# rbitr/llm.f90

Measured on AMD Instinct MI355X. Metric: tokens/sec TinyLlama-1.1B decode, higher is better.
Workload: dtype f32; 1 GPU; tinyllama f32 decode, greedy, positions 6..1140 (./llm -n 1140 -t 0); consumer=logits to host + host argmax (llmk_forward), parallelism=single GPU, seed=20260928

## Files before the change

### include/llmk.h

```cpp
#ifndef LLMK_H
#define LLMK_H

#include <stddef.h>
#include <stdint.h>

#ifdef __cplusplus
extern "C" {
#endif

#define LLMK_TYPE_F32 0
#define LLMK_TYPE_F16 1
#define LLMK_TYPE_Q4_0 2
#define LLMK_TYPE_Q6_K 14

#define LLMK_TOKEN_EMBEDDING_TABLE 0
#define LLMK_RMS_ATT_WEIGHT 1
#define LLMK_RMS_FFN_WEIGHT 2
#define LLMK_WQKV 3
#define LLMK_WO 4
#define LLMK_W13 5
#define LLMK_W2 6
#define LLMK_RMS_FINAL_WEIGHT 7
#define LLMK_WCLS 8
#define LLMK_N_TENSORS 9

#define LLMK_FLAG_NO_GRAPH 1
#define LLMK_FLAG_TIMINGS 2
#define LLMK_FLAG_MULTI_KERNEL 4

#define LLMK_OK 0
#define LLMK_E_ARG 1
#define LLMK_E_SHAPE 2
#define LLMK_E_SIZE 3
#define LLMK_E_TYPE 4
#define LLMK_E_STATE 5
#define LLMK_E_NODEVICE 6
#define LLMK_E_NOMEM 7
#define LLMK_E_TIMEOUT 8
#define LLMK_E_COMM 9
#define LLMK_E_VERIFY 10
#define LLMK_E_NONFINITE 11
#define LLMK_E_HIP 1000

typedef struct llmk_config {
    int32_t emb_dim;
    int32_t hidden_dim;
    int32_t n_layers;
    int32_t n_heads;
    int32_t n_kv_heads;
    int32_t vocab_size;
    int32_t seq_len;
    int32_t weight_type;
    int32_t device;
    int32_t flags;
} llmk_config;

typedef struct llmk_ctx llmk_ctx;

int llmk_create(const llmk_config *cfg, llmk_ctx **out);

int llmk_create_tp(const llmk_config *cfg, int tp_rank, int tp_size, llmk_ctx **out);
int llmk_tp_unique_id(char id_out[128]);
int llmk_tp_init_comm(llmk_ctx *ctx, const char id[128]);

int llmk_tp_p2p_handle(llmk_ctx *ctx, char handle_out[64]);
int llmk_tp_p2p_connect(llmk_ctx *ctx, const char *handles);
int llmk_tp_p2p_connect_local(llmk_ctx *ctx, llmk_ctx *const *ranks);
int llmk_tp_p2p_selftest(llmk_ctx *ctx, int iters);
int llmk_tp_p2p_stress(llmk_ctx *ctx, int iters, unsigned seed);
int llmk_tp_p2p_disable(llmk_ctx *ctx);

int llmk_tp_begin(llmk_ctx *ctx, int token, int pos);
int llmk_tp_segment(llmk_ctx *ctx, int seg, int layer);
int llmk_tp_read_partial(llmk_ctx *ctx, float *out);
int llmk_tp_write_partial(llmk_ctx *ctx, const float *in);
int llmk_tp_read_logits(llmk_ctx *ctx, float *out_slice);

int llmk_upload(llmk_ctx *ctx, int tensor_id, const void *host, size_t nbytes, int ggml_type);

int llmk_upload_rows(llmk_ctx *ctx, int tensor_id, int layer, int row_offset, int rows, const void *host,
                     size_t nbytes, int ggml_type);

int llmk_set_tensor_type(llmk_ctx *ctx, int tensor_id, int ggml_type);
int llmk_set_rms_eps(llmk_ctx *ctx, float eps);

int llmk_set_rope_freqs(llmk_ctx *ctx, const float *freqs, int n);

int llmk_forward(llmk_ctx *ctx, int token, int pos, float *logits_out);

int llmk_prefill(llmk_ctx* ctx, const int* tokens, int n, int pos0, float* logits_out);

int llmk_score(llmk_ctx *ctx, const int *tokens, int n, int pos0, const int *targets, float *logprob_out, int *argmax_out,
               float *logits_out);

int llmk_forward_greedy(llmk_ctx *ctx, int token, int pos, int *next_token);

typedef void (*llmk_token_fn)(int index, int token, void *user);
int llmk_decode_greedy(llmk_ctx *ctx, int token, int pos0, int n, int *ids_out, llmk_token_fn on_token, void *user);

int llmk_forward_sample(llmk_ctx *ctx, int token, int pos, float temperature, uint64_t seed, int *next_token);
int llmk_decode_sample(llmk_ctx *ctx, int token, int pos0, int n, float temperature, uint64_t seed,
                       int *ids_out, llmk_token_fn on_token, void *user);

typedef struct llmk_sampler {
    float temperature;
    int32_t top_k;
    float top_p;
    float min_p;
    uint64_t seed;
} llmk_sampler;
int llmk_forward_sample_ex(llmk_ctx *ctx, int token, int pos, const llmk_sampler *sampler, int *next_token);
int llmk_decode_sample_ex(llmk_ctx *ctx, int token, int pos0, int n, const llmk_sampler *sampler, int *ids_out,
                          llmk_token_fn on_token, void *user);
int llmk_sample_logits(llmk_ctx *ctx, const float *logits, int pos, const llmk_sampler *sampler, int *token_out, int *kept_out,
                       float *tau_out);

#define LLMK_MAX_LOGIT_BIAS 256
typedef struct llmk_logit_bias { int32_t token; float bias; } llmk_logit_bias;
typedef struct llmk_penalties {
    int32_t last_n;
    float repeat;
    float frequency;
    float presence;
    const llmk_logit_bias *bias; int32_t n_bias;
} llmk_penalties;
int llmk_set_history(llmk_ctx *ctx, const int *tokens, int n, int pos0);
int llmk_get_history(llmk_ctx *ctx, int *tokens_out, int n, int pos0);
int llmk_forward_sample_pen(llmk_ctx *ctx, int token, int pos, const llmk_sampler *sampler, const llmk_penalties *penalties, int *next_token);
int llmk_decode_sample_pen(llmk_ctx *ctx, int token, int pos0, int n, const llmk_sampler *sampler, const llmk_penalties *penalties,
                           int *ids_out, llmk_token_fn on_token, void *user);
int llmk_sample_logits_pen(llmk_ctx *ctx, const float *logits, int pos, const llmk_sampler *sampler, const llmk_penalties *penalties,
                           int *token_out, int *kept_out, float *tau_out, float *adjusted_out);

#define LLMK_MAX_TOP_LOGPROBS 20
typedef struct llmk_logprobs {
    int32_t top_n;
    float *token_logprob;
    int32_t *top_tokens;
    float *top_logprobs;
} llmk_logprobs;
int llmk_forward_sample_lp(llmk_ctx *ctx, int token, int pos, const llmk_sampler *sampler, const llmk_penalties *penalties,
                           const llmk_logprobs *logprobs, int *next_token);
int llmk_decode_sample_lp(llmk_ctx *ctx, int token, int pos0, int n, const llmk_sampler *sampler, const llmk_penalties *penalties,
                          const llmk_logprobs *logprobs, int *ids_out, llmk_token_fn on_token, void *user);
int llmk_logprob_logits(llmk_ctx *ctx, const float *logits, int token, int top_n, float *token_logprob, int32_t *top_tokens,
                        float *top_logprobs);

typedef struct llmk_batch llmk_batch;
#define LLMK_MAX_BATCH 128
int llmk_batch_create(llmk_ctx *ctx, int n_slots, int seq_len, llmk_batch **out);
int llmk_batch_destroy(llmk_batch *b);
int llmk_batch_fork(llmk_batch *b, int slot, int n_pos);
int llmk_batch_forward(llmk_batch *b, int n, const int *slots, const int *tokens, const int *pos, float *logits_out, int *argmax_out);
int llmk_batch_decode(llmk_batch *b, int n, const int *slots, const int *tokens, const int *pos0, int steps,
                      const llmk_sampler *samplers, int *ids_out);
int llmk_batch_time(llmk_batch *b, int n, int pos, int iters, float *avg_ms);

int llmk_rows_set_history(llmk_batch *b, int slot, const int *tokens, int n, int pos0);
int llmk_rows_get_history(llmk_batch *b, int slot, int *tokens_out, int n, int pos0);
int llmk_rows_decode(llmk_batch *b, int n, const int *slots, const int *tokens, const int *pos0, int steps,
                     const llmk_sampler *samplers, const llmk_penalties *penalties, const llmk_logprobs *logprobs, int *ids_out);
int llmk_rows_sample_logits(llmk_batch *b, int n, const int *slots, const int *pos, const float *logits,
                            const llmk_sampler *samplers, const llmk_penalties *penalties, const llmk_logprobs *logprobs,
                            int *tokens_out, int *kept_out, float *tau_out, float *adjusted_out);

int llmk_prefix_set(llmk_batch *b, int n_pos);
int llmk_prefix_attach(llmk_batch *b, int slot);
int llmk_prefix_len(llmk_batch *b);

int llmk_reset(llmk_ctx *ctx);

// ... 35 lines not shown
```

### llm.f90_amd/csrc/llmk.hip

```cpp
#include "../../include/llmk.h"
#include "kernels.h"
#include "token_kernel.h"
#include "prefill.h"
#include "batch.h"
#include "tp_p2p.h"

#include <rccl/rccl.h>

#include <algorithm>
#include <vector>

#include <float.h>
#include <math.h>
#include <stdio.h>
#include <stdlib.h>
#include <string.h>
#include <new>

using namespace llmk;

extern "C" int llmk_create_tp(const llmk_config* cfg, int tp_rank, int tp_size, llmk_ctx** out);
static int q16_build(llmk_ctx* c);

#define HIPCHK(expr)                                          \
    do {                                                      \
        hipError_t e_ = (expr);                               \
        if (e_ != hipSuccess) return LLMK_E_HIP + (int)e_;    \
    } while (0)

namespace {

template <class T>
hipError_t dev_alloc(T** p, size_t bytes) {
    static const bool poison = getenv("LLMK_POISON") && getenv("LLMK_POISON")[0] == '1';
    hipError_t e = hipMalloc((void**)p, bytes);
    if (e == hipSuccess && poison) {
        static thread_local hipStream_t ps = nullptr;
        if (!ps) e = hipStreamCreateWithFlags(&ps, hipStreamNonBlocking);
        if (e == hipSuccess) e = hipMemsetAsync(*p, 0xFF, bytes, ps);
        if (e == hipSuccess) e = hipStreamSynchronize(ps);
    }
    return e;
}

struct TensorDesc {
    bool layered;
    int rows;
    int K;
    bool matrix;
};

struct DevTensor {
    void* data = nullptr;
    size_t row_bytes = 0;
    int type = LLMK_TYPE_F32;
    bool uploaded = false;
    size_t rows_uploaded = 0;
    bool alias = false;
};

enum TailMode { TAIL_LOGITS, TAIL_GREEDY, TAIL_SAMPLE, TAIL_FILTER, TAIL_PENALTY, TAIL_COUNT };

template <class T>
struct DevShadow {
    T value = {};
    bool known = false;
    void invalidate() { known = false; }
    void confirm(const T& v) { value = v; known = true; }
    template <class F>
    hipError_t push(const T& want, F copy) {
        if (known && memcmp(&want, &value, sizeof(T)) == 0) return hipSuccess;
        const hipError_t e = copy();
        if (e == hipSuccess) confirm(want);
        return e;
    }
};

}

struct llmk_ctx {
    llmk_config cfg;
    int E, H, L, nh, nkv, V, S, hs, KV, kv_mul;
    int tp_rank = 0, tp_size = 1;
    int Eq, KVl, Hl, Vl, nhl;
    ncclComm_t comm = nullptr;
    unsigned long long* d_inbox = nullptr;
    unsigned* d_tp_bad = nullptr;
    TpPeers peers = {};
    void* ipc_mapped[TP_MAX_RANKS] = {};
    bool p2p = false;
    float* d_part = nullptr;
    TensorDesc gdesc[LLMK_N_TENSORS];
    TensorDesc desc[LLMK_N_TENSORS];
    DevTensor t[LLMK_N_TENSORS];
    float *d_kc = nullptr, *d_vc = nullptr;
    float *d_x = nullptr, *d_q = nullptr, *d_xb = nullptr, *d_hb = nullptr, *d_logits = nullptr, *d_rope = nullptr;
    int *d_tokpos = nullptr, *d_next = nullptr;
    int* h_tokpos = nullptr;
    float* h_logits = nullptr;
    float* h_logits_dev = nullptr;
    bool tk_direct = true;
    TkNext* h_next = nullptr;
    TkDevWords* dev_words() const { return tk_words_behind<TkDevWords>(d_logits, V); }
    TkHostWords* host_words() const { return tk_words_behind<TkHostWords>(h_logits, V); }
    TkHostWords* host_words_dev() const { return tk_words_behind<TkHostWords>(h_logits_dev, V); }
    hipStream_t stream = nullptr;
    hipGraphExec_t graph[TAIL_COUNT][2] = {};
    llmk_sample_params* h_samp = nullptr;
    DevShadow<llmk_sample_params> samp_dev = {{}, true};
    llmk_filter_params* h_filt = nullptr;
    DevShadow<llmk_filter_params> filt_dev;
    int* d_hist = nullptr;
    int* d_pen_cnt = nullptr;
    llmk_penalty_params* d_pen = nullptr;
    llmk_penalty_params* h_pen = nullptr;
    llmk_logprob_record *d_lp = nullptr, *h_lp = nullptr;
    unsigned* h_lp_top = nullptr;
    float* d_lp_raw = nullptr;
    int lp_top_n = -1;
    hipEvent_t ev[8] = {};
    float times[5] = {0, 0, 0, 0, 0};
    int n_cu = 256;
    float eps = 1e-5f;
    bool use_tk = false;
    bool tk_short_grid = false;
    bool tk_retired = false;
    int tk_range_events = 0, tk_range_run = 0;
    int tk_shape = 0;
    unsigned long long* d_gran = nullptr;
    float4* d_zeros = nullptr;
    unsigned long long* d_trace = nullptr;
    size_t tk_lds = 0;
    size_t tk_ngran = 0;
    struct PfLane {
        float *X = nullptr, *Xs = nullptr, *Q = nullptr, *XB = nullptr, *HB = nullptr, *P = nullptr, *xn = nullptr;
        unsigned* lowcnt = nullptr;
        hipStream_t stream = nullptr;
        std::vector<hipEvent_t> kv;
        hipEvent_t done = nullptr;
    } pf[2];
    int* pf_tok = nullptr;
    std::vector<int> pf_tok0;
    hipEvent_t pf_start = nullptr;
    bool pf_ready = false;
    void* up_stage[2] = {nullptr, nullptr};
    void* up_stage_dev[2] = {nullptr, nullptr};
    void* up_tmp[2] = {nullptr, nullptr};
    hipEvent_t up_done[2] = {nullptr, nullptr};
    unsigned long long* up_acc = nullptr;
    bool up_ready = false;
    void* q16[LLMK_N_TENSORS] = {};
    bool q16_dirty = true;
    bool pf_hm = false;
    unsigned* pf_flag = nullptr;
    size_t pf_pcap = 0;
    float4* sc_part[2] = {nullptr, nullptr};
    float* sc_tgt[2] = {nullptr, nullptr};
    float* sc_z[2] = {nullptr, nullptr};
    int* sc_targets = nullptr;
    float* sc_out = nullptr;
    float* h_sc = nullptr;
    float* sc_logits = nullptr;
    size_t sc_logits_cap = 0;
    bool sc_ready = false;
    int n_batches = 0;
};
typedef llmk_ctx::PfLane PfLane;

struct llmk_batch {
    llmk_ctx* ctx = nullptr;
    int n_slots = 0, seq_len = 0;
    float *d_kc = nullptr, *d_vc = nullptr;
    BdRow* d_rows = nullptr;
    int* d_tok = nullptr;
    float* d_out = nullptr;
    float* d_logits = nullptr;
    float* d_po = nullptr;
    float2* d_pml = nullptr;
    int* d_next = nullptr;
    llmk_filter_params* d_filt = nullptr;
    unsigned* d_out2 = nullptr;
    unsigned* d_err = nullptr;
    int* d_ids = nullptr;
    size_t ids_cap = 0;
    BdRow* h_rows = nullptr;
    int* h_tok = nullptr;
    llmk_filter_params* h_filt = nullptr;
    float* h_out = nullptr;
    unsigned* h_err = nullptr;
    int* d_hist = nullptr;
    int* d_pen_cnt = nullptr;
    llmk_penalty_params* d_pen = nullptr;
    llmk_penalty_params* h_pen = nullptr;
    float* d_raw = nullptr;
    llmk_logprob_record *d_lp = nullptr, *h_lp = nullptr;
    size_t lp_cap = 0;
    unsigned *d_lp_top = nullptr, *h_lp_top = nullptr;
    int P = 0, n_attached = 0;
    size_t px_cap = 0;
    float *d_pk = nullptr, *d_pv = nullptr;
    int *d_first = nullptr, *h_first = nullptr;
    int *d_colmap = nullptr, *h_colmap = nullptr;
    int pass_att = 0;
    float* d_xpo = nullptr;
    float2* d_xpml = nullptr;
};

namespace {

constexpr size_t TENSOR_SLACK = 64 * 1024;
size_t q4_row_stride(int K) { return (size_t)K / 2 + (size_t)((K / 32 + 63) / 64) * 128; }

size_t row_bytes_for(int type, int K) {
    switch (type) {
        case LLMK_TYPE_F32: return (size_t)K * 4;
        case LLMK_TYPE_F16: return (size_t)K * 2;
        case LLMK_TYPE_Q4_0: return (size_t)K / 32 * 18;
        case LLMK_TYPE_Q6_K: return (size_t)K / Q6K_WEIGHTS * Q6K_BLOCK_BYTES;
    }
    return 0;
}
size_t dev_row_bytes(int type, int K) {
    return type == LLMK_TYPE_Q4_0 ? q4_row_stride(K) : type == LLMK_TYPE_Q6_K ? q6k_row_stride(K) : row_bytes_for(type, K);
}

thread_local bool g_prepare = false;
constexpr size_t LDS_DEFAULT_LIMIT = 64 * 1024, LDS_MAX = 160 * 1024;
template <class F>
bool prepare_only(F kernel, size_t smem, hipError_t* e) {
    if (!g_prepare) return false;
    *e = smem > LDS_MAX ? hipErrorInvalidValue
       : smem > LDS_DEFAULT_LIMIT ? hipFuncSetAttribute((const void*)kernel, hipFuncAttributeMaxDynamicSharedMemorySize, (int)smem)
                                  : hipSuccess;
    return true;
}

template <int WT, int EPI, bool NORM, int ROWS, int NCH>
hipError_t launch_gemv(hipStream_t st, const GemvArgs& a) {
    const int njobs = (EPI == EPI_SWIGLU) ? a.H : a.rows / ROWS;
    const int blocks = (njobs + GEMV_WAVES - 1) / GEMV_WAVES;
    const size_t smem = 16 + (size_t)a.K * sizeof(float);
    hipError_t pe;
    if (prepare_only(gemv_kernel<WT, EPI, NORM, ROWS, NCH>, smem, &pe)) return pe;
    hipLaunchKernelGGL((gemv_kernel<WT, EPI, NORM, ROWS, NCH>), dim3(blocks), dim3(GEMV_THREADS), smem, st, a);
    return hipGetLastError();
}

template <int EPI, bool NORM>
// ... 65 lines not shown
    return with_head_size(c->hs, [&](auto hs) {
        constexpr int HS = decltype(hs)::value;
        hipError_t pe;
        if (prepare_only(attn_kernel<HS>, smem, &pe)) return pe;
        hipLaunchKernelGGL((attn_kernel<HS>), dim3(c->nhl), dim3(256), smem, c->stream, c->d_q, kc, vc, c->d_xb, c->d_tokpos, c->KVl, c->kv_mul);
        return hipGetLastError();
    });
}

GemvArgs base_args(llmk_ctx* c, int tid, int l, const float* x, const float* norm_w, float* y) {
    GemvArgs a;
    memset(&a, 0, sizeof(a));
    const DevTensor& t = c->t[tid];
    const TensorDesc& d = c->desc[tid];
    const size_t lrows = d.layered ? (size_t)l * d.rows : 0;
    a.W = (const char*)t.data + lrows * t.row_bytes;
    a.row_stride = (int)t.row_bytes;
    a.eps = c->eps;
    a.x = x;
    a.norm_w = norm_w;
    a.y = y;
    a.rows = d.rows;
    a.K = d.K;
    a.rope_freqs = c->d_rope;
    a.tokpos = c->d_tokpos;
    a.E = c->Eq;
    a.KV = c->KVl;
    a.hs = c->hs;
    a.H = c->Hl;
    return a;
}

hipError_t launch_qkv(llmk_ctx* c, int l) {
    GemvArgs a = base_args(c, LLMK_WQKV, l, c->d_x, (const float*)c->t[LLMK_RMS_ATT_WEIGHT].data + (size_t)l * c->E, c->d_q);
    a.kc = c->d_kc + (size_t)l * c->S * c->KVl;
    a.vc = c->d_vc + (size_t)l * c->S * c->KVl;
    return launch_gemv_t<EPI_ROPE_KV, true>(c->cfg.weight_type, c->stream, a, c->n_cu);
}
hipError_t launch_wo(llmk_ctx* c, int l) {
    if (c->tp_size > 1 || c->comm || c->p2p) {
        GemvArgs a = base_args(c, LLMK_WO, l, c->d_xb, nullptr, c->d_part);
        return launch_gemv_t<EPI_STORE, false>(c->cfg.weight_type, c->stream, a, c->n_cu);
    }
    GemvArgs a = base_args(c, LLMK_WO, l, c->d_xb, nullptr, c->d_x);
    return launch_gemv_t<EPI_RESID, false>(c->cfg.weight_type, c->stream, a, c->n_cu);
}
hipError_t launch_w13(llmk_ctx* c, int l) {
    GemvArgs a = base_args(c, LLMK_W13, l, c->d_x, (const float*)c->t[LLMK_RMS_FFN_WEIGHT].data + (size_t)l * c->E, c->d_hb);
    return launch_gemv_t<EPI_SWIGLU, true>(c->cfg.weight_type, c->stream, a, c->n_cu);
}
hipError_t launch_w2(llmk_ctx* c, int l) {
    if (c->tp_size > 1 || c->comm || c->p2p) {
        GemvArgs a = base_args(c, LLMK_W2, l, c->d_hb, nullptr, c->d_part);
        return launch_gemv_t<EPI_STORE, false>(c->cfg.weight_type, c->stream, a, c->n_cu);
    }
    GemvArgs a = base_args(c, LLMK_W2, l, c->d_hb, nullptr, c->d_x);
    return launch_gemv_t<EPI_RESID, false>(c->cfg.weight_type, c->stream, a, c->n_cu);
}
hipError_t launch_cls(llmk_ctx* c) {
    GemvArgs a = base_args(c, LLMK_WCLS, 0, c->d_x, (const float*)c->t[LLMK_RMS_FINAL_WEIGHT].data,
                           c->d_logits + (size_t)c->tp_rank * c->Vl);
    if (c->t[LLMK_WCLS].type == LLMK_TYPE_Q6_K) {
        const size_t smem = 16 + (size_t)a.K * sizeof(float);
        const int blocks = (a.rows + GEMV_WAVES * Q6K_RPW - 1) / (GEMV_WAVES * Q6K_RPW);
        hipError_t pe;
        if (prepare_only(gemv_q6k_kernel<true>, smem, &pe)) return pe;
        hipLaunchKernelGGL((gemv_q6k_kernel<true>), dim3(blocks), dim3(GEMV_THREADS), smem, c->stream, a);
        return hipGetLastError();
    }
    return launch_gemv_t<EPI_STORE, true>(c->t[LLMK_WCLS].type, c->stream, a, c->n_cu);
}
hipError_t launch_embed(llmk_ctx* c) {
    hipLaunchKernelGGL(embed_kernel, dim3((c->E + 255) / 256), dim3(256), 0, c->stream,
                       (const float*)c->t[LLMK_TOKEN_EMBEDDING_TABLE].data, c->d_tokpos, c->d_x, c->E);
    return hipGetLastError();
}

#define HIPRET(expr)                     \
    do {                                 \
        hipError_t e_ = (expr);          \
        if (e_ != hipSuccess) return e_; \
    } while (0)

struct TkGreedy { int gflags = 0, id_index = 0; };
template <class TK>
hipError_t launch_token_kernel_t(llmk_ctx* c, bool direct, const TkGreedy& g) {
    TokenArgs a;
    a.gflags = g.gflags | ((TK_DEBUG && getenv("LLMK_TK_NOSYNC")) ? TKG_NOSYNC : 0);
    a.emb = (const float*)c->t[LLMK_TOKEN_EMBEDDING_TABLE].data;
    a.rms = (const float*)c->t[LLMK_RMS_ATT_WEIGHT].data;
    a.wqkv = TK::Q4 ? c->q16[LLMK_WQKV] : c->t[LLMK_WQKV].data;
    a.wo = TK::Q4 ? c->q16[LLMK_WO] : c->t[LLMK_WO].data;
    a.w13 = TK::Q4 ? c->q16[LLMK_W13] : c->t[LLMK_W13].data;
    a.w2 = TK::Q4 ? c->q16[LLMK_W2] : c->t[LLMK_W2].data;
    a.wcls = (TK::Q4 && !TK::CLSQ6) ? c->q16[LLMK_WCLS] : c->t[LLMK_WCLS].data;
    a.kc = c->d_kc;
    a.vc = c->d_vc;
    a.rope = c->d_rope;
    a.tokpos = (direct || g.gflags) ? nullptr : c->d_tokpos;
    a.tok_imm = (g.gflags & TKG_CAND_IN) ? g.id_index : c->h_tokpos[0];
    a.pos_imm = c->h_tokpos[1];
    a.serial_imm = c->h_tokpos[2];
    a.g_qkv = c->d_gran;
    a.logits = direct ? c->h_logits_dev : c->d_logits;
    a.err = &c->dev_words()->err;
    a.herr = (direct || g.gflags) ? &c->host_words_dev()->err : nullptr;
    a.zeros = c->d_zeros;
#ifdef LLMK_TK_DEBUG
    a.trace = c->d_trace;
#endif
    a.L = c->L;
    a.S = c->S;
    a.eps = c->eps;
    const dim3 grid((TK_DEBUG && c->tk_short_grid) ? TK_NCU - 1 : TK_NCU);
    if (g.gflags) hipLaunchKernelGGL((token_kernel<TK, true>), grid, dim3(TK_THREADS), c->tk_lds, c->stream, a);
    else hipLaunchKernelGGL((token_kernel<TK>), grid, dim3(TK_THREADS), c->tk_lds, c->stream, a);
    return hipGetLastError();
}
#ifndef LLMK_TK_EXTRA_SHAPES
#define LLMK_TK_EXTRA_SHAPES(X)
#endif
#define LLMK_TK_SHAPES(X)                                                                                          \
    X(TkTinyLlama) X(TkSmall) X(TkTinyLlamaF16) X(TkSmallF16) X(TkLlama7BQ4) X(TkTinyLlamaQ4) X(TkLlama7BQ4Q6)     \
    X(TkTinyLlamaQ4Q6) X(TkLlama7BF16) X(TkMistral7BQ4Q6) LLMK_TK_EXTRA_SHAPES(X)
struct TkEntry {
    int E, H, NH, NKV, V, WT, CLS;
    bool q4;
    hipError_t (*launch)(llmk_ctx*, bool, const TkGreedy&);
    int (*setup)(llmk_ctx*, int);
};
template <class TK> int tk_setup(llmk_ctx* c, int id);
#define TK_ENTRY(...) {__VA_ARGS__::E, __VA_ARGS__::H, __VA_ARGS__::NH, __VA_ARGS__::NKV, __VA_ARGS__::V, __VA_ARGS__::WT, __VA_ARGS__::CLS, \
                       __VA_ARGS__::Q4, launch_token_kernel_t<__VA_ARGS__>, tk_setup<__VA_ARGS__>},
static const TkEntry tk_table[] = {LLMK_TK_SHAPES(TK_ENTRY)};
#undef TK_ENTRY
constexpr int TK_NSHAPES = (int)(sizeof(tk_table) / sizeof(tk_table[0]));
hipError_t launch_token_kernel(llmk_ctx* c, bool direct = false, const TkGreedy& g = TkGreedy()) {
    if (c->tk_shape < 1 || c->tk_shape > TK_NSHAPES) return hipErrorInvalidValue;
    return tk_table[c->tk_shape - 1].launch(c, direct, g);
}
__global__ __launch_bounds__(64) void cand_resolve_kernel(const float2* __restrict__ cand, int* id_out, int* next, unsigned* err, int V) {
    float bv;
    int bi;
    cand_fold(cand, TK_NCU, bv, bi);
    if (threadIdx.x == 0) {
        const bool none = (unsigned)bi >= (unsigned)V;
        const unsigned e = *err;
        if (none && e == 0) atomicOr(err, 0x2000u);
        if (!none && e == 0) {
            next[0] = bi + 1;
            __hip_atomic_store(id_out, bi + 1, __ATOMIC_RELAXED, __HIP_MEMORY_SCOPE_SYSTEM);
        }
    }
}

template <class TK>
int tk_setup(llmk_ctx* c, int id) {
    const llmk_config& g = c->cfg;
    if (c->use_tk || g.emb_dim != TK::E || g.hidden_dim != TK::H || g.n_heads != TK::NH || g.n_kv_heads != TK::NKV ||
        g.vocab_size != TK::V || g.weight_type != TK::WT || c->t[LLMK_WCLS].type != TK::CLS)
        return LLMK_OK;
    const size_t lds = ((size_t)TkLds<TK>::ATT_S + 2 * (size_t)c->S * sizeof(float) + 15) & ~(size_t)15;
    c->tk_lds = lds < 96 * 1024 ? 96 * 1024 : lds;
    if (c->tk_lds > 160 * 1024) return LLMK_OK;
    HIPCHK(hipFuncSetAttribute((const void*)token_kernel<TK>, hipFuncAttributeMaxDynamicSharedMemorySize, (int)c->tk_lds));
    HIPCHK(hipFuncSetAttribute((const void*)token_kernel<TK, true>, hipFuncAttributeMaxDynamicSharedMemorySize, (int)c->tk_lds));
    int per_cu = 0;
    HIPCHK(hipOccupancyMaxActiveBlocksPerMultiprocessor(&per_cu, token_kernel<TK>, TK_THREADS, c->tk_lds));
    if (per_cu < 1 || (long long)per_cu * c->n_cu < TK_NCU) return LLMK_OK;
    static_assert(tk_qsc_front<TK>() == (size_t)TK::QKV + 3 * (size_t)TK::E + TK::H + (size_t)TK::NH * (TkAttPlan<TK>::PMAX - 1) * (TK::HS + 2),
                  "tk_qsc_front: the attention parts are TkAttPlan's");
    const size_t ngran = tk_qsc_front<TK>() + TK_QSC_GRANULES;
    c->tk_ngran = ngran;
    if (!c->d_gran) HIPCHK(dev_alloc(&c->d_gran, ngran * sizeof(unsigned long long)));
    if (!c->d_zeros) HIPCHK(dev_alloc(&c->d_zeros, (size_t)TK_NCU * TK_WAVES * 1024));
    if (TK_DEBUG && getenv("LLMK_TK_TRACE")) HIPCHK(dev_alloc(&c->d_trace, (size_t)TK_NCU * TK_TRACE_N * 8));
    HIPCHK(hipMemset(c->d_gran, 0, ngran * sizeof(unsigned long long)));
    HIPCHK(hipMemset(c->d_zeros, 0, (size_t)TK_NCU * TK_WAVES * 1024));
    c->use_tk = true;
    c->tk_shape = id;
    return LLMK_OK;
}

int tk_setup_all(llmk_ctx* c) {
    if ((c->cfg.flags & (LLMK_FLAG_MULTI_KERNEL | LLMK_FLAG_TIMINGS)) || c->n_cu != TK_NCU || c->tp_size != 1 || c->tk_retired) return LLMK_OK;
    int rc = LLMK_OK;
    for (int i = 0; i < TK_NSHAPES && rc == LLMK_OK; ++i) rc = tk_table[i].setup(c, i + 1);
// ... 109 lines not shown
    else hipLaunchKernelGGL(tp_allreduce_add_kernel<false>, grid, block, 0, c->stream, c->peers, c->d_part, c->d_x, c->d_tokpos, call,
                            2 * c->L, c->tp_rank, c->tp_size, c->E, err, 0u);
    return hipGetLastError();
}
hipError_t launch_tp_allgather(llmk_ctx* c, unsigned jseed = 0) {
    const dim3 grid((c->V + 255) / 256), block(256);
    unsigned* err = &c->dev_words()->err;
    if (jseed) hipLaunchKernelGGL(tp_allgather_kernel<true>, grid, block, 0, c->stream, c->peers, c->d_logits, c->d_tokpos, 2 * c->L,
                                  c->tp_rank, c->tp_size, c->E, c->V, err, jseed);
    else hipLaunchKernelGGL(tp_allgather_kernel<false>, grid, block, 0, c->stream, c->peers, c->d_logits, c->d_tokpos, 2 * c->L,
                            c->tp_rank, c->tp_size, c->E, c->V, err, 0u);
    return hipGetLastError();
}

hipError_t enqueue_token(llmk_ctx* c, TailMode tail, bool timed) {
    HIPRET(hipMemcpyAsync(c->d_tokpos, c->h_tokpos, 4 * sizeof(int), hipMemcpyHostToDevice, c->stream));
    if (c->p2p) {
        HIPRET(launch_embed(c));
        for (int l = 0; l < c->L; ++l) {
            HIPRET(launch_qkv(c, l));
            HIPRET(launch_attn(c, l));
            HIPRET(launch_wo(c, l));
            HIPRET(launch_tp_allreduce_add(c, 2 * l));
            HIPRET(launch_w13(c, l));
            HIPRET(launch_w2(c, l));
            HIPRET(launch_tp_allreduce_add(c, 2 * l + 1));
        }
        HIPRET(launch_cls(c));
        HIPRET(launch_tp_allgather(c));
        return enqueue_tail(c, tail);
    }
    if (c->use_tk) {
        HIPRET(launch_token_kernel(c));
        return enqueue_tail(c, tail);
    }
    HIPRET(launch_embed(c));
    for (int l = 0; l < c->L; ++l) {
        if (timed) HIPRET(hipEventRecord(c->ev[0], c->stream));
        HIPRET(launch_qkv(c, l));
        if (timed) HIPRET(hipEventRecord(c->ev[1], c->stream));
        HIPRET(launch_attn(c, l));
        if (timed) HIPRET(hipEventRecord(c->ev[2], c->stream));
        HIPRET(launch_wo(c, l));
        HIPRET(launch_w13(c, l));
        HIPRET(launch_w2(c, l));
        if (timed) {
            HIPRET(hipEventRecord(c->ev[3], c->stream));
            HIPRET(hipEventSynchronize(c->ev[3]));
            float ms;
            HIPRET(hipEventElapsedTime(&ms, c->ev[0], c->ev[1])); c->times[0] += ms;
            HIPRET(hipEventElapsedTime(&ms, c->ev[1], c->ev[2])); c->times[2] += ms;
            HIPRET(hipEventElapsedTime(&ms, c->ev[2], c->ev[3])); c->times[3] += ms;
        }
    }
    if (timed) HIPRET(hipEventRecord(c->ev[4], c->stream));
    HIPRET(launch_cls(c));
    if (timed) {
        HIPRET(hipEventRecord(c->ev[5], c->stream));
        HIPRET(hipEventSynchronize(c->ev[5]));
        float ms;
        HIPRET(hipEventElapsedTime(&ms, c->ev[4], c->ev[5])); c->times[4] += ms;
    }
    return enqueue_tail(c, tail);
}

void drop_graphs(llmk_ctx* c) {
    for (auto& per_tail : c->graph)
        for (hipGraphExec_t& g : per_tail)
            if (g) { hipGraphExecDestroy(g); g = nullptr; }
}
int build_graph(llmk_ctx* c, TailMode tail, hipGraphExec_t* out) {
    hipGraph_t g = nullptr;
    HIPCHK(hipStreamBeginCapture(c->stream, hipStreamCaptureModeThreadLocal));
    hipError_t e = enqueue_token(c, tail, false);
    hipError_t e2 = hipStreamEndCapture(c->stream, &g);
    if (e != hipSuccess) { if (g) hipGraphDestroy(g); return LLMK_E_HIP + (int)e; }
    HIPCHK(e2);
    e = hipGraphInstantiate(out, g, nullptr, nullptr, 0);
    hipGraphDestroy(g);
    HIPCHK(e);
    return LLMK_OK;
}

int check_ready(llmk_ctx* c) {
    if (!c) return LLMK_E_ARG;
    for (int i = 0; i < LLMK_N_TENSORS; ++i)
        if (!c->t[i].uploaded) return LLMK_E_STATE;
    if (c->use_tk && tk_table[c->tk_shape - 1].q4 && c->q16_dirty) return q16_build(c);
    return LLMK_OK;
}

constexpr int TK_RANGE_LIMIT = 4;
bool tk_inject_timeout(int pos) {
    const char* at = TK_DEBUG ? getenv("LLMK_TK_INJECT_TIMEOUT") : nullptr;
    return at && atoi(at) == pos;
}
int tk_clear_err(llmk_ctx* c) {
    HIPCHK(hipMemsetAsync(&c->dev_words()->err, 0, sizeof(unsigned), c->stream));
    HIPCHK(hipStreamSynchronize(c->stream));
    c->host_words()->err = 0;
    c->h_next->err = 0;
    return LLMK_OK;
}
bool tk_range_only(unsigned code) { return (code & 0x4000u) != 0 && (code & 0x2f00u) == 0; }
int tk_retire(llmk_ctx* c, unsigned code, int pos) {
    int rc = tk_clear_err(c);
    if (rc) return rc;
    c->use_tk = false;
    c->tk_retired = true;
    drop_graphs(c);
    for (int i = 0; i < LLMK_N_TENSORS; ++i)
        if (c->q16[i]) { hipFree(c->q16[i]); c->q16[i] = nullptr; }
    c->q16_dirty = true;
    const char* what = (code & 0x2000u) ? "found no finite logit among its candidates"
                     : (code & 0x4000u) ? "met an activation beyond the f16 range of its matrix-core operands"
                                        : "timed out waiting for its peer workgroups";
    fprintf(stderr, "llmk: the persistent token kernel %s (code 0x%x, position %d); this context continues on the multi-kernel path\n", what, code, pos);
    return LLMK_OK;
}

const char* tp_describe_err(const llmk_ctx* c, unsigned code, char* buf, size_t n) {
    if ((code >> 28) != 3u) { snprintf(buf, n, "code 0x%x", code); return buf; }
    const unsigned per = 2u * (unsigned)c->L + 1u, e24 = code & 0xffffffu;
    const unsigned cur = (unsigned)c->h_tokpos[2] * per + per;
    unsigned epoch = (cur & ~0xffffffu) | e24;
    if (epoch > cur) epoch -= 0x1000000u;
    const unsigned serial = (epoch - 1u) / per, call = (epoch - 1u) % per;
    if (call == per - 1u) snprintf(buf, n, "code 0x%x: rank %u's logits slice never arrived (all-gather of serial %u)", code, (code >> 24) & 15u, serial);
    else snprintf(buf, n, "code 0x%x: rank %u's partial never arrived (all-reduce %u of serial %u: layer %u, %s)", code, (code >> 24) & 15u,
                  call, serial, call / 2u, (call & 1u) ? "w2" : "wo");
    return buf;
}
int run_token_pass(llmk_ctx* c, int token, int pos, TailMode tail) {
    int rc = check_ready(c);
    if (rc) return rc;
    if (token < 1 || token > c->V || pos < 1 || pos > c->S) return LLMK_E_ARG;
    HIPCHK(hipSetDevice(c->cfg.device));
    c->h_tokpos[0] = token - 1;
    c->h_tokpos[1] = pos;
    const bool timed = (c->cfg.flags & LLMK_FLAG_TIMINGS) != 0;
    for (int attempt = 0; attempt < 2; ++attempt) {
        c->h_tokpos[2] += 1;
        c->tk_short_grid = c->use_tk && tk_inject_timeout(pos);
        if ((c->tp_size > 1 || c->comm) && !c->p2p) {
            rc = enqueue_token_tp(c);
            if (rc) return rc;
            HIPCHK(enqueue_tail(c, tail));
        } else if (timed || (c->cfg.flags & LLMK_FLAG_NO_GRAPH)) {
            HIPCHK(enqueue_token(c, tail, timed));
        } else if (c->use_tk && tail == TAIL_LOGITS && c->tk_direct) {
            c->host_words()->err = 0;
            HIPCHK(launch_token_kernel(c, true));
        } else {
            hipGraphExec_t* g = &c->graph[tail][c->lp_top_n >= 0 ? 1 : 0];
            if (!*g) {
                rc = build_graph(c, tail, g);
                if (rc) return rc;
            }
            HIPCHK(hipGraphLaunch(*g, c->stream));
        }
        HIPCHK(hipStreamSynchronize(c->stream));
        if (c->p2p) {
            const unsigned perr = tail != TAIL_LOGITS ? c->h_next->err : c->host_words()->err;
            char what[160];
            if (perr) fprintf(stderr, "llmk: rank %d of %d: a peer's granules never arrived (%s; position %d, serial %d)\n",
                              c->tp_rank, c->tp_size, tp_describe_err(c, perr, what, sizeof(what)), pos, c->h_tokpos[2]);
            return perr ? LLMK_E_TIMEOUT : LLMK_OK;
        }
        if (!c->use_tk) return LLMK_OK;
        const unsigned err = tail != TAIL_LOGITS ? c->h_next->err : c->host_words()->err;
        if (err == 0) { c->tk_range_run = 0; return LLMK_OK; }
        if (tk_range_only(err) && c->tk_range_run + 1 < TK_RANGE_LIMIT) {
            ++c->tk_range_run;
            if (c->tk_range_events++ == 0)
                fprintf(stderr, "llmk: position %d holds an activation beyond the f16 range of the persistent q4_0 kernel's operands (code 0x%x): that "
                                "position is redone on the multi-kernel path, the kernel stays in use\n", pos, err);
            rc = tk_clear_err(c);
            if (rc) return rc;
            c->use_tk = false;
            const hipError_t e = enqueue_token(c, tail, false);
            c->use_tk = true;
            HIPCHK(e);
            HIPCHK(hipStreamSynchronize(c->stream));
            return LLMK_OK;
        }
        rc = tk_retire(c, err, pos);
        if (rc) return rc;
    }
    return LLMK_E_TIMEOUT;
}
int run_token(llmk_ctx* c, int token, int pos, TailMode tail) {
    const bool filt = tail == TAIL_FILTER || tail == TAIL_PENALTY, samp = tail == TAIL_SAMPLE;
    if (filt) c->filt_dev.invalidate();
    if (samp) c->samp_dev.invalidate();
    const int rc = run_token_pass(c, token, pos, tail);
    if (rc == LLMK_OK && filt) c->filt_dev.confirm(*c->h_filt);
    if (rc == LLMK_OK && samp) c->samp_dev.confirm(*c->h_samp);
    return rc;
}

#ifndef LLMK_PF_H_STEP1
#define LLMK_PF_H_STEP1 1.00
#define LLMK_PF_H_STEP2 1.32
#define LLMK_PF_HQ_STEP1 1.20
#define LLMK_PF_HQ_STEP2 1.92
#endif
struct PfPlan { int nr, nk, total, U, grid; };
PfPlan pf_plan(const llmk_ctx* c, int rows, int K, int T = PF_TMAX, int wt = -1) {
    if (wt < 0) wt = c->cfg.weight_type;
    static const double step_f32[2] = {2.45, 4.25}, step_h[2] = {LLMK_PF_H_STEP1, LLMK_PF_H_STEP2}, step_hq[2] = {LLMK_PF_HQ_STEP1, LLMK_PF_HQ_STEP2};
    static const double step_q8[2] = {LLMK_PF_HQ_STEP1, LLMK_PF_HQ_STEP2 * 0.925};
    static const double step_q6[2] = {LLMK_PF_HQ_STEP1 * 1.3, LLMK_PF_HQ_STEP2 * 1.3};
    const bool q6 = wt == LLMK_TYPE_Q6_K;
    const double* step_us = !c->pf_hm ? step_f32 : wt == LLMK_TYPE_F16 ? step_h : q6 ? step_q6
                            : (wt == LLMK_TYPE_Q4_0 && (T + 15) / 16 == 8) ? step_q8 : step_hq;
    PfPlan best{};
    double best_t = 1e30;
    for (int nr = 1; nr <= 2; ++nr) {
// ... 436 lines not shown
    if (E % nh || nh % nkv) return LLMK_E_SHAPE;
    const int hs = E / nh;
    if (hs != 16 && hs != 32 && hs != 64 && hs != 128) return LLMK_E_SHAPE;
    if (E % 32 || H % 32 || (V & 1)) return LLMK_E_SHAPE;
    const int kalign = cfg->weight_type == LLMK_TYPE_Q4_0 ? 32 : cfg->weight_type == LLMK_TYPE_F16 ? 8 : 4;
    if (nkv % tp_size || H % tp_size || V % tp_size || (H / tp_size) % kalign || ((V / tp_size) & 1)) return LLMK_E_SHAPE;
    if (((nh / tp_size) * hs) % kalign || (((nkv / tp_size) * hs) & 1)) return LLMK_E_SHAPE;
    if (cfg->weight_type != LLMK_TYPE_F32 && cfg->weight_type != LLMK_TYPE_F16 && cfg->weight_type != LLMK_TYPE_Q4_0)
        return LLMK_E_TYPE;
    int ndev = 0;
    if (hipGetDeviceCount(&ndev) != hipSuccess || ndev <= 0) return LLMK_E_NODEVICE;
    if (cfg->device < 0 || cfg->device >= ndev) return LLMK_E_NODEVICE;
    HIPCHK(hipSetDevice(cfg->device));

    llmk_ctx* c = new (std::nothrow) llmk_ctx();
    if (!c) return LLMK_E_NOMEM;
    c->cfg = *cfg;
    c->E = E; c->H = H; c->L = L; c->nh = nh; c->nkv = nkv; c->V = V; c->S = S;
    c->hs = hs; c->KV = nkv * hs; c->kv_mul = nh / nkv;
    c->tp_rank = tp_rank; c->tp_size = tp_size;
    c->nhl = nh / tp_size; c->Eq = c->nhl * hs; c->KVl = (nkv / tp_size) * hs; c->Hl = H / tp_size; c->Vl = V / tp_size;
    hipDeviceProp_t prop;
    if (hipGetDeviceProperties(&prop, cfg->device) == hipSuccess && prop.multiProcessorCount > 0)
        c->n_cu = prop.multiProcessorCount;

    const int KV = c->KV;
    c->gdesc[LLMK_TOKEN_EMBEDDING_TABLE] = {false, V, E, false};
    c->gdesc[LLMK_RMS_ATT_WEIGHT] = {true, 1, E, false};
    c->gdesc[LLMK_RMS_FFN_WEIGHT] = {true, 1, E, false};
    c->gdesc[LLMK_WQKV] = {true, E + 2 * KV, E, true};
    c->gdesc[LLMK_WO] = {true, E, E, true};
    c->gdesc[LLMK_W13] = {true, 2 * H, E, true};
    c->gdesc[LLMK_W2] = {true, E, H, true};
    c->gdesc[LLMK_RMS_FINAL_WEIGHT] = {false, 1, E, false};
    c->gdesc[LLMK_WCLS] = {false, V, E, true};
    for (int i = 0; i < LLMK_N_TENSORS; ++i) c->desc[i] = c->gdesc[i];
    c->desc[LLMK_WQKV] = {true, c->Eq + 2 * c->KVl, E, true};
    c->desc[LLMK_WO] = {true, E, c->Eq, true};
    c->desc[LLMK_W13] = {true, 2 * c->Hl, E, true};
    c->desc[LLMK_W2] = {true, E, c->Hl, true};
    c->desc[LLMK_WCLS] = {false, c->Vl, E, true};

    int rc = LLMK_OK;
#define CK(expr)                                                        \
    do {                                                                \
        hipError_t e_ = (expr);                                         \
        if (e_ != hipSuccess && rc == LLMK_OK) rc = LLMK_E_HIP + (int)e_; \
    } while (0)
    for (int i = 0; i < LLMK_N_TENSORS && rc == LLMK_OK; ++i) {
        const TensorDesc& d = c->desc[i];
        DevTensor& t = c->t[i];
        t.type = d.matrix ? cfg->weight_type : LLMK_TYPE_F32;
        const size_t rows = (size_t)d.rows * (d.layered ? L : 1);
        t.row_bytes = dev_row_bytes(t.type, d.K);
        if (i == LLMK_RMS_FFN_WEIGHT || i == LLMK_RMS_FINAL_WEIGHT) {
            t.alias = true;
            t.data = (char*)c->t[LLMK_RMS_ATT_WEIGHT].data + (size_t)(i == LLMK_RMS_FFN_WEIGHT ? L : 2 * L) * E * sizeof(float);
            continue;
        }
        const size_t extra = i == LLMK_RMS_ATT_WEIGHT ? ((size_t)L + 1) * E * sizeof(float) : 0;
        CK(dev_alloc(&t.data, rows * t.row_bytes + extra + TENSOR_SLACK));
        if (rc == LLMK_OK) {
            if (t.type == LLMK_TYPE_Q4_0) CK(hipMemset(t.data, 0, rows * t.row_bytes + TENSOR_SLACK));
            else CK(hipMemset((char*)t.data + rows * t.row_bytes + extra, 0, TENSOR_SLACK));
        }
    }
    const size_t kvn = (size_t)L * S * c->KVl;
    CK(dev_alloc(&c->d_kc, kvn * sizeof(float)));
    CK(dev_alloc(&c->d_vc, kvn * sizeof(float)));
    CK(dev_alloc(&c->d_x, (size_t)E * sizeof(float)));
    CK(dev_alloc(&c->d_q, (size_t)E * sizeof(float)));
    CK(dev_alloc(&c->d_xb, (size_t)E * sizeof(float)));
    CK(dev_alloc(&c->d_hb, (size_t)H * sizeof(float)));
    CK(dev_alloc(&c->d_part, (size_t)E * sizeof(float)));
    const size_t logits_bytes = (size_t)V * sizeof(float) + sizeof(TkDevWords);
    CK(dev_alloc(&c->d_logits, logits_bytes));
    CK(dev_alloc(&c->d_rope, (size_t)(hs / 2) * sizeof(float)));
    CK(dev_alloc(&c->d_tokpos, 4 * sizeof(int)));
    CK(dev_alloc(&c->d_next, 2 * sizeof(int)));
    CK(hipHostMalloc(&c->h_tokpos, 4 * sizeof(int), hipHostMallocDefault));
    CK(hipHostMalloc(&c->h_logits, (size_t)V * sizeof(float) + sizeof(TkHostWords) + (size_t)S * sizeof(int), hipHostMallocMapped));
    CK(hipHostGetDevicePointer((void**)&c->h_logits_dev, c->h_logits, 0));
    c->tk_direct = !(getenv("LLMK_TK_DIRECT") && getenv("LLMK_TK_DIRECT")[0] == '0');
    CK(hipHostMalloc(&c->h_next, sizeof(TkNext), hipHostMallocDefault));
    CK(hipHostMalloc(&c->h_samp, sizeof(llmk_sample_params), hipHostMallocDefault));
    CK(hipHostMalloc(&c->h_filt, sizeof(llmk_filter_params), hipHostMallocDefault));
    CK(hipStreamCreateWithFlags(&c->stream, hipStreamNonBlocking));
    for (int i = 0; i < 8; ++i) CK(hipEventCreate(&c->ev[i]));
    if (rc == LLMK_OK) rc = tk_setup_all(c);
    if (rc == LLMK_OK) {
        g_prepare = true;
        hipError_t pe = launch_qkv(c, 0);
        if (pe == hipSuccess) pe = launch_attn(c, 0);
        if (pe == hipSuccess) pe = launch_wo(c, 0);
        if (pe == hipSuccess) pe = launch_w13(c, 0);
        if (pe == hipSuccess) pe = launch_w2(c, 0);
        if (pe == hipSuccess) pe = launch_cls(c);
        g_prepare = false;
        if (pe == hipErrorInvalidValue) rc = LLMK_E_SHAPE;
        else CK(pe);
    }
    if (rc == LLMK_OK) {
        CK(hipMemset(c->d_logits, 0, logits_bytes));
        c->h_tokpos[0] = 0; c->h_tokpos[1] = 0; c->h_tokpos[2] = 0; c->h_tokpos[3] = 0;
        CK(hipMemset(c->d_kc, 0, kvn * sizeof(float)));
        CK(hipMemset(c->d_vc, 0, kvn * sizeof(float)));
        CK(hipMemset(c->d_x, 0, (size_t)E * sizeof(float)));
        CK(hipMemset(c->d_q, 0, (size_t)E * sizeof(float)));
        CK(hipMemset(c->d_xb, 0, (size_t)E * sizeof(float)));
        CK(hipMemset(c->d_hb, 0, (size_t)H * sizeof(float)));
        float fr[64];
        for (int j = 0; j < hs / 2; ++j) fr[j] = 1.0f / powf(10000.0f, (float)(2 * j + 1) / (float)hs);
        CK(hipMemcpy(c->d_rope, fr, (size_t)(hs / 2) * sizeof(float), hipMemcpyHostToDevice));
        CK(hipDeviceSynchronize());
    }
#undef CK
    if (rc != LLMK_OK) {
        llmk_destroy(c);
        return rc;
    }
    *out = c;
    return LLMK_OK;
}

constexpr size_t UP_STAGE_BYTES = (size_t)8 << 20;
__global__ void sum16_kernel(const unsigned* __restrict__ w, size_t nbytes, unsigned long long* out) {
    const size_t nwords = nbytes / 4;
    unsigned long long t = 0;
    for (size_t i = (size_t)blockIdx.x * blockDim.x + threadIdx.x; i < nwords; i += (size_t)gridDim.x * blockDim.x) {
        const unsigned v = w[i];
        t += (v & 0xffffu) + (v >> 16);
    }
    if (blockIdx.x == 0 && threadIdx.x == 0 && (nbytes & 2)) t += reinterpret_cast<const unsigned short*>(w)[nbytes / 2 - 1];
    for (int o = 32; o > 0; o >>= 1) t += __shfl_xor(t, o, 64);
    if ((threadIdx.x & 63) == 0) atomicAdd(out, t);
}
static unsigned long long stage_rows(uint8_t* dst, const uint8_t* src, size_t spitch, size_t col_bytes, size_t nrows) {
    unsigned long long t = 0;
    for (size_t r = 0; r < nrows; ++r) {
        const uint16_t* p = reinterpret_cast<const uint16_t*>(src + r * spitch);
        uint16_t* q = reinterpret_cast<uint16_t*>(dst + r * col_bytes);
        unsigned long long a = 0;
        for (size_t i = 0; i < col_bytes / 2; ++i) { const uint16_t v = p[i]; q[i] = v; a += v; }
        t += a;
    }
    return t;
}
__global__ void stage_copy_kernel(const unsigned* __restrict__ src, unsigned* __restrict__ dst, size_t nwords) {
    for (size_t i = (size_t)blockIdx.x * blockDim.x + threadIdx.x; i < nwords; i += (size_t)gridDim.x * blockDim.x) dst[i] = src[i];
}
static bool verify_uploads() {
    static const bool on = !(getenv("LLMK_VERIFY_UPLOAD") && getenv("LLMK_VERIFY_UPLOAD")[0] == '0');
    return on;
}
static hipError_t device_sum16(const void* dev, size_t nbytes, unsigned long long* d_acc, unsigned long long* out) {
    hipError_t e = hipMemsetAsync(d_acc, 0, sizeof(*d_acc), 0);
    if (e != hipSuccess) return e;
    hipLaunchKernelGGL(sum16_kernel, dim3(512), dim3(256), 0, 0, (const unsigned*)dev, nbytes, d_acc);
    e = hipGetLastError();
    if (e == hipSuccess) e = hipMemcpy(out, d_acc, sizeof(*out), hipMemcpyDeviceToHost);
    return e;
}

static int q16_build(llmk_ctx* c) {
    static const int mats[5] = {LLMK_WQKV, LLMK_WO, LLMK_W13, LLMK_W2, LLMK_WCLS};
    for (int i = 0; i < 5; ++i) {
// ... 84 lines not shown
                                    n * col_bytes / 4);
            e = hipGetLastError();
            if (e == hipSuccess) e = hipEventRecord(c->up_done[b], 0);
            if (e != hipSuccess) rc = LLMK_E_HIP + (int)e;
        }
        if (rc != LLMK_OK || !verify) break;
#ifdef LLMK_TK_DEBUG
        {
            static const int inject = getenv("LLMK_UPLOAD_INJECT") ? atoi(getenv("LLMK_UPLOAD_INJECT")) : 0;
            static bool first_block = true;
            if (first_block && attempt <= inject) (void)hipMemsetAsync(dst0, 0xA5, 64, 0);
            if (attempt >= inject) first_block = false;
        }
#endif
        unsigned long long got = 0;
        const hipError_t e = device_sum16(dst0, (size_t)nrows * t.row_bytes, d_acc, &got);
        if (e != hipSuccess) { rc = LLMK_E_HIP + (int)e; break; }
        if (got == want) break;
        fprintf(stderr, "llmk: upload of tensor %d, layer %d, local rows %zu..%zu (%zu bytes) did not arrive intact: 16-bit word sum 0x%llx on the "
                        "device, 0x%llx on the host (attempt %d of 3)%s\n", tid, layer, first_row, first_row + (size_t)nrows - 1, (size_t)nrows * col_bytes,
                got, want, attempt, attempt < 3 ? " -- staging it again" : "");
        if (attempt == 3) rc = LLMK_E_VERIFY;
    }
    if (rc == LLMK_OK) { const hipError_t e = hipDeviceSynchronize(); if (e != hipSuccess) rc = LLMK_E_HIP + (int)e; }
    if (rc) return rc;
    t.rows_uploaded += (size_t)nrows;
    if (t.rows_uploaded >= (size_t)d.rows * (d.layered ? c->L : 1)) t.uploaded = true;
    return LLMK_OK;
}

static int upload_rows_sharded(llmk_ctx* c, int tid, int layer, int row0, int nrows, const uint8_t* src, int type) {
    const TensorDesc& g = c->gdesc[tid];
    const size_t pitch = row_bytes_for(type, g.K);
    const int r = c->tp_rank, E = c->E, KV = c->KV, H = c->H;
    struct Run { int gfirst, n, lfirst; };
    Run runs[3];
    int nruns = 0;
    size_t col_off = 0, col_bytes = pitch;
    switch (tid) {
        case LLMK_WQKV:
            runs[nruns++] = {r * c->Eq, c->Eq, 0};
            runs[nruns++] = {E + r * c->KVl, c->KVl, c->Eq};
            runs[nruns++] = {E + KV + r * c->KVl, c->KVl, c->Eq + c->KVl};
            break;
        case LLMK_WO:
            runs[nruns++] = {0, E, 0};
            col_off = row_bytes_for(type, r * c->Eq); col_bytes = row_bytes_for(type, c->Eq);
            break;
        case LLMK_W13:
            runs[nruns++] = {r * c->Hl, c->Hl, 0};
            runs[nruns++] = {H + r * c->Hl, c->Hl, c->Hl};
            break;
        case LLMK_W2:
            runs[nruns++] = {0, E, 0};
            col_off = row_bytes_for(type, r * c->Hl); col_bytes = row_bytes_for(type, c->Hl);
            break;
        case LLMK_WCLS:
            runs[nruns++] = {r * c->Vl, c->Vl, 0};
            break;
        default:
            runs[nruns++] = {0, g.rows, 0};
            break;
    }
    for (int i = 0; i < nruns; ++i) {
        const int a = std::max(runs[i].gfirst, row0), b = std::min(runs[i].gfirst + runs[i].n, row0 + nrows);
        if (a >= b) continue;
        const int rc = upload_block(c, tid, layer, runs[i].lfirst + (a - runs[i].gfirst), b - a, src + (size_t)(a - row0) * pitch, pitch,
                                    col_off, col_bytes);
        if (rc) return rc;
    }
    return LLMK_OK;
}

int llmk_upload_rows(llmk_ctx* c, int tid, int layer, int row_offset, int rows, const void* host, size_t nbytes,
                     int ggml_type) {
    if (!c || !host || tid < 0 || tid >= LLMK_N_TENSORS) return LLMK_E_ARG;
    const TensorDesc& g = c->gdesc[tid];
    DevTensor& t = c->t[tid];
    const int nl = g.layered ? c->L : 1;
    if (layer < 0 || layer >= nl || row_offset < 0 || rows <= 0 || row_offset + rows > g.rows) return LLMK_E_ARG;
    if (ggml_type != t.type) return LLMK_E_TYPE;
    if (nbytes != (size_t)rows * row_bytes_for(ggml_type, g.K)) return LLMK_E_SIZE;
    HIPCHK(hipSetDevice(c->cfg.device));
    if (c->tp_size > 1) return upload_rows_sharded(c, tid, layer, row_offset, rows, (const uint8_t*)host, ggml_type);
    const size_t pitch = row_bytes_for(ggml_type, g.K);
    return upload_block(c, tid, layer, row_offset, rows, (const uint8_t*)host, pitch, 0, pitch);
}

int llmk_upload(llmk_ctx* c, int tid, const void* host, size_t nbytes, int ggml_type) {
    if (!c || !host || tid < 0 || tid >= LLMK_N_TENSORS) return LLMK_E_ARG;
    const TensorDesc& g = c->gdesc[tid];
    const int nl = g.layered ? c->L : 1;
    if (ggml_type != c->t[tid].type) return LLMK_E_TYPE;
    const size_t per_layer = (size_t)g.rows * row_bytes_for(ggml_type, g.K);
    if (nbytes != per_layer * nl) return LLMK_E_SIZE;
    c->t[tid].rows_uploaded = 0;
    c->t[tid].uploaded = false;
    for (int l = 0; l < nl; ++l) {
        int rc = llmk_upload_rows(c, tid, l, 0, g.rows, (const char*)host + (size_t)l * per_layer, per_layer, ggml_type);
        if (rc) return rc;
    }
    return LLMK_OK;
}

int llmk_set_tensor_type(llmk_ctx* c, int tid, int ggml_type) {
    if (!c || tid != LLMK_WCLS) return LLMK_E_ARG;
    if (ggml_type != LLMK_TYPE_F32 && ggml_type != LLMK_TYPE_F16 && ggml_type != LLMK_TYPE_Q4_0 && ggml_type != LLMK_TYPE_Q6_K) return LLMK_E_TYPE;
    DevTensor& t = c->t[tid];
    if (t.type == ggml_type) return LLMK_OK;
    const TensorDesc& d = c->desc[tid];
    const int kalign = ggml_type == LLMK_TYPE_Q6_K ? Q6K_WEIGHTS : ggml_type == LLMK_TYPE_Q4_0 ? 32 : ggml_type == LLMK_TYPE_F16 ? 8 : 4;
    if (d.K % kalign) return LLMK_E_SHAPE;
    HIPCHK(hipSetDevice(c->cfg.device));
    HIPCHK(hipStreamSynchronize(c->stream));
    if (t.data) HIPCHK(hipFree(t.data));
    if (c->pf_ready) pf_teardown(c);
    t.data = nullptr;
    t.type = ggml_type;
    t.uploaded = false;
    t.rows_uploaded = 0;
    const size_t rows = (size_t)d.rows * (d.layered ? c->L : 1);
    t.row_bytes = dev_row_bytes(ggml_type, d.K);
    HIPCHK(dev_alloc(&t.data, rows * t.row_bytes + TENSOR_SLACK));
    HIPCHK(hipMemset(t.data, 0, rows * t.row_bytes + TENSOR_SLACK));
    if (c->q16[tid]) { HIPCHK(hipFree(c->q16[tid])); c->q16[tid] = nullptr; }
    c->q16_dirty = true;
    if (c->use_tk) {
        c->use_tk = false;
        drop_graphs(c);
    }
    { const int rc = tk_setup_all(c); if (rc) return rc; }
    g_prepare = true;
    const hipError_t pe = launch_cls(c);
    g_prepare = false;
    if (pe == hipErrorInvalidValue) return LLMK_E_SHAPE;
    HIPCHK(pe);
    return LLMK_OK;
}

int llmk_set_rms_eps(llmk_ctx* c, float eps) {
    if (!c || !(eps > 0.f) || !(eps < 1.f)) return LLMK_E_ARG;
    HIPCHK(hipSetDevice(c->cfg.device));
    HIPCHK(hipStreamSynchronize(c->stream));
    c->eps = eps;
    drop_graphs(c);
    return LLMK_OK;
}

int llmk_set_rope_freqs(llmk_ctx* c, const float* freqs, int n) {
    if (!c || !freqs || n != c->hs / 2) return LLMK_E_ARG;
    HIPCHK(hipSetDevice(c->cfg.device));
    HIPCHK(hipMemcpy(c->d_rope, freqs, (size_t)n * sizeof(float), hipMemcpyHostToDevice));
    return LLMK_OK;
}

int llmk_forward(llmk_ctx* c, int token, int pos, float* logits_out) {
    if (!c || !logits_out) return LLMK_E_ARG;
    int rc = run_token(c, token, pos, TAIL_LOGITS);
    if (rc) return rc;
    memcpy(logits_out, c->h_logits, (size_t)c->V * sizeof(float));
    return LLMK_OK;
}

int llmk_prefill(llmk_ctx* c, const int* tokens, int n, int pos0, float* logits_out) {
    if (!c || !tokens || !logits_out || n < 1 || pos0 < 1 || pos0 + n - 1 > c->S) return LLMK_E_ARG;
    int rc = check_ready(c);
    if (rc) return rc;
    for (int i = 0; i < n; ++i)
        if (tokens[i] < 1 || tokens[i] > c->V) return LLMK_E_ARG;
    if (!pf_eligible(c)) {
        for (int i = 0; i < n; ++i) {
            rc = run_token(c, tokens[i], pos0 + i, TAIL_LOGITS);
            if (rc) return rc;
        }
        memcpy(logits_out, c->h_logits, (size_t)c->V * sizeof(float));
        return LLMK_OK;
    }
    HIPCHK(hipSetDevice(c->cfg.device));
    rc = pf_setup(c, true);
    if (rc) return rc;
    rc = pf_run(c, tokens, n, pos0, nullptr);
    if (rc) return rc;
    HIPCHK(launch_cls(c));
    HIPCHK(hipMemcpyAsync(c->h_logits, c->d_logits, (size_t)c->V * sizeof(float), hipMemcpyDeviceToHost, c->stream));
    HIPCHK(hipStreamSynchronize(c->stream));
    if (pf_flagged(c)) {
        static bool told = false;
        return pf_redo(c, "llmk_prefill", &told, [&] { return llmk_prefill(c, tokens, n, pos0, logits_out); });
    }
    memcpy(logits_out, c->h_logits, (size_t)c->V * sizeof(float));
    return LLMK_OK;
}

int llmk_score(llmk_ctx* c, const int* tokens, int n, int pos0, const int* targets, float* logprob_out, int* argmax_out, float* logits_out) {
    if (!c || !tokens || n < 1 || pos0 < 1 || pos0 + n - 1 > c->S) return LLMK_E_ARG;
    if ((!logprob_out && !argmax_out && !logits_out) || (logprob_out && !targets)) return LLMK_E_ARG;
    int rc = check_ready(c);
    if (rc) return rc;
    for (int i = 0; i < n; ++i)
        if (tokens[i] < 1 || tokens[i] > c->V || (targets && (targets[i] < 0 || targets[i] > c->V))) return LLMK_E_ARG;
    HIPCHK(hipSetDevice(c->cfg.device));
    rc = sc_setup(c);
    if (rc) return rc;
    const int V = c->V;
    ScoreJob sj{logprob_out != nullptr, logits_out != nullptr, n, ScPlan{0, 0, 0}};
    bool batched = pf_eligible(c);
    if (batched) {
        rc = pf_setup(c, true);
        if (rc) return rc;
        const int ct = c->t[LLMK_WCLS].type;
        sj.sp = sc_plan(c, std::min(n, (int)PF_TMAX));
        if (ct != LLMK_TYPE_Q6_K && sj.sp.R == 0) {
            batched = false;
            static bool told_slow = false;
            if (!told_slow) {
                told_slow = true;
                fprintf(stderr, "llmk: llmk_score runs token by token on this context: %s\n",
                        V % 4 ? "vocab_size is not a multiple of 4 (the classifier GEMM's partial tiles are read as 4-row vectors)"
                              : "no 128-row chunk of the classifier fits the prefill's partial-tile workspace");
            }
        }
    }
    if (batched && sj.want_logits && c->sc_logits_cap < (size_t)n) {
        if (c->sc_logits) { hipFree(c->sc_logits); c->sc_logits = nullptr; c->sc_logits_cap = 0; }
        HIPCHK(dev_alloc(&c->sc_logits, (size_t)n * V * sizeof(float)));
        c->sc_logits_cap = (size_t)n;
    }
    std::vector<int> tg0;
    if (sj.want_lp) {
        tg0.assign(targets, targets + n);
        for (int& t : tg0) --t;
        HIPCHK(hipMemcpyAsync(c->sc_targets, tg0.data(), (size_t)n * sizeof(int), hipMemcpyHostToDevice, c->stream));
    }
    if (!batched) {
        const int np = (V + PF_SC_ROWS - 1) / PF_SC_ROWS;
        PfEpiArgs e;
        memset(&e, 0, sizeof(e));
        for (int i = 0; i < n; ++i) {
            rc = run_token(c, tokens[i], pos0 + i, TAIL_LOGITS);
            if (rc) return rc;
            if (logits_out) memcpy(logits_out + (size_t)i * V, c->h_logits, (size_t)V * sizeof(float));
            PfScoreArgs s;
            memset(&s, 0, sizeof(s));
// ... 271 lines not shown
}
int llmk_forward_sample(llmk_ctx* c, int token, int pos, float temperature, uint64_t seed, int* next_token) {
    if (!c || !next_token) return LLMK_E_ARG;
    const llmk_sampler sp = {temperature, 0, 1.f, 0.f, seed};
    return sample_forward(c, token, pos, &sp, nullptr, next_token);
}
int llmk_forward_sample_ex(llmk_ctx* c, int token, int pos, const llmk_sampler* sp, int* next_token) {
    if (!c || !next_token) return LLMK_E_ARG;
    return sample_forward(c, token, pos, sp, nullptr, next_token);
}
int llmk_forward_sample_pen(llmk_ctx* c, int token, int pos, const llmk_sampler* sp, const llmk_penalties* pn, int* next_token) {
    if (!c || !next_token || !pn || token < 1 || token > c->V || pos < 1 || pos > c->S) return LLMK_E_ARG;
    return sample_forward(c, token, pos, sp, pn, next_token);
}
int llmk_decode_greedy(llmk_ctx* c, int token, int pos0, int n, int* ids_out, llmk_token_fn on_token, void* user) {
    if (!decode_args_ok(c, token, pos0, n, ids_out)) return LLMK_E_ARG;
    return decode_run(c, token, pos0, n, TAIL_GREEDY, ids_out, on_token, user);
}
int llmk_decode_sample(llmk_ctx* c, int token, int pos0, int n, float temperature, uint64_t seed, int* ids_out,
                       llmk_token_fn on_token, void* user) {
    if (!decode_args_ok(c, token, pos0, n, ids_out)) return LLMK_E_ARG;
    const llmk_sampler sp = {temperature, 0, 1.f, 0.f, seed};
    return sample_decode(c, token, pos0, n, &sp, nullptr, ids_out, on_token, user);
}
int llmk_decode_sample_ex(llmk_ctx* c, int token, int pos0, int n, const llmk_sampler* sp, int* ids_out, llmk_token_fn on_token, void* user) {
    if (!decode_args_ok(c, token, pos0, n, ids_out)) return LLMK_E_ARG;
    return sample_decode(c, token, pos0, n, sp, nullptr, ids_out, on_token, user);
}
int llmk_decode_sample_pen(llmk_ctx* c, int token, int pos0, int n, const llmk_sampler* sp, const llmk_penalties* pn, int* ids_out,
                           llmk_token_fn on_token, void* user) {
    if (!decode_args_ok(c, token, pos0, n, ids_out) || !pn) return LLMK_E_ARG;
    return sample_decode(c, token, pos0, n, sp, pn, ids_out, on_token, user);
}
int llmk_sample_logits(llmk_ctx* c, const float* logits, int pos, const llmk_sampler* sp, int* token_out_, int* kept_out, float* tau_out) {
    if (!c || !logits || !token_out_ || pos < 1 || c->tp_size != 1) return LLMK_E_ARG;
    return sample_logits(c, logits, pos, sp, nullptr, token_out_, kept_out, tau_out, nullptr);
}
int llmk_sample_logits_pen(llmk_ctx* c, const float* logits, int pos, const llmk_sampler* sp, const llmk_penalties* pn, int* token_out_,
                           int* kept_out, float* tau_out, float* adjusted_out) {
    if (!c || !logits || !token_out_ || !pn || pos < 1 || pos > c->S || c->tp_size != 1) return LLMK_E_ARG;
    return sample_logits(c, logits, pos, sp, pn, token_out_, kept_out, tau_out, adjusted_out);
}
int llmk_forward_sample_lp(llmk_ctx* c, int token, int pos, const llmk_sampler* sp, const llmk_penalties* pn, const llmk_logprobs* lp,
                           int* next_token) {
    if (!c || !next_token || !logprob_args_ok(c, lp) || (!sp && pn) || token < 1 || token > c->V || pos < 1 || pos > c->S) return LLMK_E_ARG;
    int rc = check_ready(c);
    if (rc) return rc;
    LpScope scope{c};
    TailMode tail = TAIL_GREEDY;
    rc = sp ? sampler_request(c, sp, pn, &tail, lp) : logprob_request(c, lp, false);
    if (rc == LLMK_OK) rc = token_out(c, token, pos, tail, next_token);
    if (rc == LLMK_OK) logprob_deliver(c, lp, 0, c->S);
    return rc;
}
int llmk_decode_sample_lp(llmk_ctx* c, int token, int pos0, int n, const llmk_sampler* sp, const llmk_penalties* pn, const llmk_logprobs* lp,
                          int* ids_out, llmk_token_fn on_token, void* user) {
    if (!decode_args_ok(c, token, pos0, n, ids_out) || !logprob_args_ok(c, lp) || (!sp && pn)) return LLMK_E_ARG;
    int rc = check_ready(c);
    if (rc) return rc;
    LpScope scope{c};
    TailMode tail = TAIL_GREEDY;
    rc = sp ? sampler_request(c, sp, pn, &tail, lp) : logprob_request(c, lp, false);
    return rc ? rc : decode_run(c, token, pos0, n, tail, ids_out, on_token, user, lp);
}
int llmk_logprob_logits(llmk_ctx* c, const float* logits, int token, int top_n, float* token_logprob, int32_t* top_tokens, float* top_logprobs) {
    const llmk_logprobs lp = {top_n, token_logprob, top_tokens, top_logprobs};
    if (!c || !logits || !logprob_args_ok(c, &lp) || token < 0 || token > c->V) return LLMK_E_ARG;
    int rc = check_ready(c);
    if (rc) return rc;
    if ((rc = lp_setup(c, false)) != LLMK_OK) return rc;
    *c->h_lp_top = (unsigned)top_n;
    HIPCHK(hipMemcpyAsync(c->d_logits, logits, (size_t)c->V * sizeof(float), hipMemcpyHostToDevice, c->stream));
    HIPCHK(copy_logprob_top(c));
    HIPCHK(enqueue_logprob(c, c->d_logits, nullptr, nullptr, 0, token, c->d_lp + c->S));
    HIPCHK(hipMemcpyAsync(c->h_lp + c->S, c->d_lp + c->S, sizeof(llmk_logprob_record), hipMemcpyDeviceToHost, c->stream));
    HIPCHK(hipStreamSynchronize(c->stream));
    logprob_deliver(c, &lp, 0, c->S);
    return LLMK_OK;
}
int llmk_set_history(llmk_ctx* c, const int* tokens, int n, int pos0) {
    if (!c || !tokens || n < 1 || pos0 < 1 || pos0 + n - 1 > c->S) return LLMK_E_ARG;
    for (int i = 0; i < n; ++i)
        if (tokens[i] < 0 || tokens[i] > c->V) return LLMK_E_ARG;
    const int rc = pen_setup(c);
    if (rc) return rc;
    HIPCHK(hipMemcpyAsync(c->d_hist + (pos0 - 1), tokens, (size_t)n * sizeof(int), hipMemcpyHostToDevice, c->stream));
    HIPCHK(hipStreamSynchronize(c->stream));
    return LLMK_OK;
}
int llmk_get_history(llmk_ctx* c, int* tokens_out, int n, int pos0) {
    if (!c || !tokens_out || n < 1 || pos0 < 1 || pos0 + n - 1 > c->S) return LLMK_E_ARG;
    const int rc = pen_setup(c);
    if (rc) return rc;
    HIPCHK(hipMemcpyAsync(tokens_out, c->d_hist + (pos0 - 1), (size_t)n * sizeof(int), hipMemcpyDeviceToHost, c->stream));
    HIPCHK(hipStreamSynchronize(c->stream));
    return LLMK_OK;
}

static_assert(LLMK_MAX_BATCH == PF_TMAX, "a batch's rows are the rows of one prefill pass");
constexpr size_t bd_attn_smem(int hs) { return ((size_t)BD_WAVES * 16 * hs + 2 * BD_WAVES * 16) * sizeof(float); }

static void batch_free(llmk_batch* b) {
    void* dev[] = {b->d_kc, b->d_vc, b->d_rows, b->d_tok, b->d_out, b->d_logits, b->d_po, b->d_pml, b->d_next, b->d_filt, b->d_out2, b->d_err, b->d_ids,
                   b->d_hist, b->d_pen_cnt, b->d_pen, b->d_raw, b->d_lp, b->d_lp_top, b->d_pk, b->d_pv, b->d_first, b->d_colmap, b->d_xpo, b->d_xpml};
    for (void* p : dev)
        if (p) hipFree(p);
    void* host[] = {b->h_rows, b->h_tok, b->h_filt, b->h_out, b->h_err, b->h_pen, b->h_lp, b->h_lp_top, b->h_first, b->h_colmap};
    for (void* p : host)
        if (p) hipHostFree(p);
    delete b;
}

static hipError_t bd_pass(llmk_batch* b, int n, int max_pos, bool want_logits, const ScPlan& sp, int step = 0) {
    llmk_ctx* c = b->ctx;
    PfLane& w = c->pf[0];
    const int E = c->E, KV = c->KV, QKV = E + 2 * KV, T = n;
    const BdCaches bc{b->d_rows, (size_t)b->seq_len * KV, b->n_slots, b->seq_len};
    int parts = bd_parts(n, c->nkv, max_pos, c->n_cu), tpp = bd_tiles_per_part(max_pos, parts);
    const bool shared = b->pass_att > 0;
    int groups = 0, pparts = 0, ptpp = 0;
    if (shared) {
        int own = 0;
        for (int i = 0; i < n; ++i) {
            const int pos = b->h_rows[i].pos + step;
            own = std::max(own, (pos + BD_TILE - 1) / BD_TILE - b->h_first[b->h_rows[i].slot] / BD_TILE);
        }
        parts = bd_parts(n, c->nkv, own * BD_TILE, c->n_cu);
        tpp = bd_tiles_per_part(own * BD_TILE, parts);
        groups = bd_prefix_groups(b->pass_att, c->kv_mul);
        pparts = bd_prefix_parts(b->pass_att, c->nkv, c->kv_mul, b->P, c->n_cu);
        ptpp = bd_tiles_per_part(b->P, pparts);
    }
    PfEpiArgs e;
    HIPRET(pf_layers(c, w, b->d_tok, T, 0, (const float*)c->t[LLMK_RMS_FINAL_WEIGHT].data, e, [&](int l, PfEpiArgs& a) -> hipError_t {
        float* kc = b->d_kc + (size_t)l * b->n_slots * bc.slot_stride;
        float* vc = b->d_vc + (size_t)l * b->n_slots * bc.slot_stride;
        a.kc = kc; a.vc = vc;
        hipLaunchKernelGGL(bd_epi_qkv_kernel, dim3((QKV / 4 + 255) / 256, T), dim3(256), 0, w.stream, a, bc);
        HIPRET(hipGetLastError());
        return with_head_size(c->hs, [&](auto hs) {
            constexpr int HS = decltype(hs)::value;
            if (shared) {
                const int np = pparts + parts;
                const size_t px = (size_t)l * b->P * KV;
                hipLaunchKernelGGL((bd_attn_prefix_kernel<HS>), dim3(c->nkv, groups, pparts), dim3(BD_WAVES * WAVE), bd_attn_smem(HS), w.stream,
                                   w.Q, b->d_pk + px, b->d_pv + px, b->d_xpo, b->d_xpml, b->d_colmap, T, b->P, KV, c->kv_mul, E, ptpp, np);
                HIPRET(hipGetLastError());
                hipLaunchKernelGGL((bd_attn_own_kernel<HS>), dim3(c->nkv, T, parts), dim3(BD_WAVES * WAVE), bd_attn_smem(HS), w.stream,
                                   w.Q, kc, vc, b->d_xpo, b->d_xpml, bc, b->d_first, KV, c->kv_mul, E, tpp, np, pparts);
                HIPRET(hipGetLastError());
                hipLaunchKernelGGL((bd_attn_fold_kernel<HS>), dim3(c->nkv, T), dim3(256), 0, w.stream, b->d_xpo, b->d_xpml, w.XB, bc, b->d_first,
                                   c->kv_mul, E, np, pparts);
                return hipGetLastError();
            }
            hipLaunchKernelGGL((bd_attn_kernel<HS>), dim3(c->nkv, T, parts), dim3(BD_WAVES * WAVE), bd_attn_smem(HS), w.stream,
                               w.Q, kc, vc, w.XB, b->d_po, b->d_pml, bc, KV, c->kv_mul, E, tpp);
            HIPRET(hipGetLastError());
            if (parts > 1) hipLaunchKernelGGL((bd_attn_merge_kernel<HS>), dim3(c->nkv, T), dim3(256), 0, w.stream, b->d_po, b->d_pml, w.XB, bc, c->kv_mul, E, parts);
            return hipGetLastError();
        });
    }));
    ScoreJob sj{false, want_logits, n, sp};
    sj.out = b->d_out;
    sj.logits = b->d_logits;
    return sc_batch(c, w, 0, e, sj, T, 0);
}

static int bd_ready(llmk_batch* b, ScPlan* sp, int rows) {
    llmk_ctx* c = b->ctx;
    int rc = check_ready(c);
    if (rc) return rc;
    HIPCHK(hipSetDevice(c->cfg.device));
    if ((rc = sc_setup(c)) != LLMK_OK) return rc;
    if ((rc = pf_setup(c, true)) != LLMK_OK) return rc;
// ... 8 lines not shown
    for (int i = 0; i < n; ++i) {
        if (slots[i] < 0 || slots[i] >= b->n_slots || seen[slots[i]]) return false;
        seen[slots[i]] = true;
        if (fed && (tokens[i] < 1 || tokens[i] > b->ctx->V)) return false;
        if (pos[i] < 1 || pos[i] > b->seq_len || span - 1 > b->seq_len - pos[i]) return false;
        if (b->n_attached > 0 && pos[i] <= b->h_first[slots[i]]) return false;
    }
    return true;
}
static hipError_t bd_upload_rows(llmk_batch* b, int n, const int* slots, const int* tokens, const int* pos) {
    for (int i = 0; i < n; ++i) {
        b->h_rows[i] = BdRow{slots[i], pos[i]};
        b->h_tok[i] = tokens ? tokens[i] - 1 : 0;
    }
    hipStream_t st = b->ctx->stream;
    b->pass_att = 0;
    if (b->n_attached > 0) {
        for (int i = 0; i < n; ++i)
            if (b->h_first[slots[i]] > 0) b->h_colmap[b->pass_att++] = i;
        if (b->pass_att > 0) {
            const int rg = bd_prefix_rg(b->ctx->kv_mul), cells = bd_prefix_groups(b->pass_att, b->ctx->kv_mul) * rg;
            for (int k = b->pass_att; k < cells; ++k) b->h_colmap[k] = -1;
            HIPRET(hipMemcpyAsync(b->d_colmap, b->h_colmap, (size_t)cells * sizeof(int), hipMemcpyHostToDevice, st));
        }
    }
    HIPRET(hipMemcpyAsync(b->d_rows, b->h_rows, (size_t)n * sizeof(BdRow), hipMemcpyHostToDevice, st));
    return hipMemcpyAsync(b->d_tok, b->h_tok, (size_t)n * sizeof(int), hipMemcpyHostToDevice, st);
}
static hipError_t bd_fetch_flag(llmk_ctx* c) {
    unsigned* h_flag = &c->host_words()->pf_flag;
    *h_flag = 0;
    return c->pf_hm ? hipMemcpyAsync(h_flag, c->pf_flag, sizeof(unsigned), hipMemcpyDeviceToHost, c->stream) : hipSuccess;
}

int llmk_batch_create(llmk_ctx* c, int n_slots, int seq_len, llmk_batch** out) {
    if (!c || !out || n_slots < 1 || n_slots > LLMK_MAX_BATCH || seq_len < 1 || seq_len > c->S) return LLMK_E_ARG;
    *out = nullptr;
    int rc = check_ready(c);
    if (rc) return rc;
    if (!pf_shape_ok(c) || c->kv_mul > BD_MAX_GROUP) return LLMK_E_SHAPE;
    HIPCHK(hipSetDevice(c->cfg.device));
    llmk_batch* b = new llmk_batch;
    b->ctx = c; b->n_slots = n_slots; b->seq_len = seq_len;
    ScPlan sp;
    if ((rc = bd_ready(b, &sp, n_slots)) != LLMK_OK) { delete b; return rc; }
    const size_t cache = (size_t)c->L * n_slots * seq_len * c->KV * sizeof(float), nb = LLMK_MAX_BATCH;
    auto alloc = [&]() -> int {
        HIPCHK(dev_alloc(&b->d_kc, cache));
        HIPCHK(dev_alloc(&b->d_vc, cache));
        HIPCHK(hipMemsetAsync(b->d_kc, 0, cache, c->stream));
        HIPCHK(hipMemsetAsync(b->d_vc, 0, cache, c->stream));
        HIPCHK(dev_alloc(&b->d_rows, nb * sizeof(BdRow)));
        HIPCHK(dev_alloc(&b->d_tok, nb * sizeof(int)));
        HIPCHK(dev_alloc(&b->d_out, 2 * nb * sizeof(float)));
        HIPCHK(dev_alloc(&b->d_logits, (size_t)n_slots * c->V * sizeof(float)));
        HIPCHK(dev_alloc(&b->d_po, (size_t)c->n_cu * BD_MAX_GROUP * c->hs * sizeof(float)));
        HIPCHK(dev_alloc(&b->d_pml, (size_t)c->n_cu * BD_MAX_GROUP * sizeof(float2)));
        HIPCHK(dev_alloc(&b->d_next, nb * sizeof(int)));
        HIPCHK(dev_alloc(&b->d_filt, nb * sizeof(llmk_filter_params)));
        HIPCHK(dev_alloc(&b->d_out2, 2 * nb * sizeof(unsigned)));
        HIPCHK(dev_alloc(&b->d_err, sizeof(unsigned)));
        HIPCHK(hipHostMalloc(&b->h_rows, nb * sizeof(BdRow), hipHostMallocDefault));
        HIPCHK(hipHostMalloc(&b->h_tok, nb * sizeof(int), hipHostMallocDefault));
        HIPCHK(hipHostMalloc(&b->h_filt, nb * sizeof(llmk_filter_params), hipHostMallocDefault));
        HIPCHK(hipHostMalloc(&b->h_out, 2 * nb * sizeof(float), hipHostMallocDefault));
        HIPCHK(hipHostMalloc(&b->h_err, sizeof(unsigned), hipHostMallocDefault));
        HIPCHK(with_head_size(c->hs, [](auto hs) {
            constexpr int HS = decltype(hs)::value;
            return hipFuncSetAttribute((const void*)bd_attn_kernel<HS>, hipFuncAttributeMaxDynamicSharedMemorySize, (int)bd_attn_smem(HS));
        }));
        HIPCHK(hipStreamSynchronize(c->stream));
        return LLMK_OK;
    };
    if ((rc = alloc()) != LLMK_OK) { batch_free(b); return rc; }
    ++c->n_batches;
    *out = b;
    return LLMK_OK;
}

int llmk_batch_destroy(llmk_batch* b) {
    if (!b) return LLMK_E_ARG;
    llmk_ctx* c = b->ctx;
    hipSetDevice(c->cfg.device);
    hipStreamSynchronize(c->stream);
    --c->n_batches;
    batch_free(b);
    return LLMK_OK;
}

static hipError_t prefix_first(llmk_batch* b, int slot, int first) {
    b->n_attached += (first > 0) - (b->h_first[slot] > 0);
    b->h_first[slot] = first;
    return hipMemcpyAsync(b->d_first + slot, b->h_first + slot, sizeof(int), hipMemcpyHostToDevice, b->ctx->stream);
}

int llmk_batch_fork(llmk_batch* b, int slot, int n_pos) {
    if (!b || slot < 0 || slot >= b->n_slots || n_pos < 0 || n_pos > std::min(b->seq_len, b->ctx->S)) return LLMK_E_ARG;
    llmk_ctx* c = b->ctx;
    HIPCHK(hipSetDevice(c->cfg.device));
    const size_t row = (size_t)c->KV, slot_rows = (size_t)b->seq_len * row;
    float* caches[2][2] = {{b->d_kc, c->d_kc}, {b->d_vc, c->d_vc}};
    for (auto& p : caches)
        for (int l = 0; l < c->L; ++l) {
            float* dst = p[0] + ((size_t)l * b->n_slots + slot) * slot_rows;
            if ((size_t)n_pos < (size_t)b->seq_len)
                HIPCHK(hipMemsetAsync(dst + (size_t)n_pos * row, 0, (slot_rows - (size_t)n_pos * row) * sizeof(float), c->stream));
            if (n_pos > 0)
                HIPCHK(hipMemcpyAsync(dst, p[1] + (size_t)l * c->S * row, (size_t)n_pos * row * sizeof(float), hipMemcpyDeviceToDevice, c->stream));
        }
    if (b->d_hist) HIPCHK(hipMemsetAsync(b->d_hist + (size_t)slot * b->seq_len, 0, (size_t)b->seq_len * sizeof(int), c->stream));
    if (b->h_first && b->h_first[slot] > 0) HIPCHK(prefix_first(b, slot, 0));
    HIPCHK(hipStreamSynchronize(c->stream));
    return LLMK_OK;
}

int llmk_prefix_set(llmk_batch* b, int n_pos) {
    if (!b || n_pos < 0 || n_pos > std::min(b->seq_len, b->ctx->S) - 1) return LLMK_E_ARG;
    if (b->n_attached > 0) return LLMK_E_STATE;
    llmk_ctx* c = b->ctx;
    if (n_pos == 0) { b->P = 0; return LLMK_OK; }
    int rc = check_ready(c);
    if (rc) return rc;
    HIPCHK(hipSetDevice(c->cfg.device));
    const size_t row = (size_t)c->KV, nb = LLMK_MAX_BATCH;
    const size_t states = nb * c->nkv * 2 * BD_MAX_PARTS * c->kv_mul, words = (size_t)b->n_slots * sizeof(int);
    if (!b->d_first) {
        HIPCHK(dev_alloc(&b->d_first, words));
        HIPCHK(hipMemsetAsync(b->d_first, 0, words, c->stream));
    }
    if (!b->h_first) {
        HIPCHK(hipHostMalloc(&b->h_first, words, hipHostMallocDefault));
        memset(b->h_first, 0, words);
    }
    if (!b->d_colmap) HIPCHK(dev_alloc(&b->d_colmap, (nb + BD_MAX_GROUP) * sizeof(int)));
    if (!b->h_colmap) HIPCHK(hipHostMalloc(&b->h_colmap, (nb + BD_MAX_GROUP) * sizeof(int), hipHostMallocDefault));
    if (!b->d_xpo) HIPCHK(dev_alloc(&b->d_xpo, states * c->hs * sizeof(float)));
    if (!b->d_xpml) HIPCHK(dev_alloc(&b->d_xpml, states * sizeof(float2)));
    HIPCHK(with_head_size(c->hs, [](auto hs) -> hipError_t {
        constexpr int HS = decltype(hs)::value;
        HIPRET(hipFuncSetAttribute((const void*)bd_attn_prefix_kernel<HS>, hipFuncAttributeMaxDynamicSharedMemorySize, (int)bd_attn_smem(HS)));
        return hipFuncSetAttribute((const void*)bd_attn_own_kernel<HS>, hipFuncAttributeMaxDynamicSharedMemorySize, (int)bd_attn_smem(HS));
    }));
    if (b->px_cap < (size_t)n_pos) {
        HIPCHK(hipStreamSynchronize(c->stream));
        if (b->d_pk) { hipFree(b->d_pk); b->d_pk = nullptr; }
        if (b->d_pv) { hipFree(b->d_pv); b->d_pv = nullptr; }
        b->px_cap = 0; b->P = 0;
        HIPCHK(dev_alloc(&b->d_pk, (size_t)c->L * n_pos * row * sizeof(float)));
        HIPCHK(dev_alloc(&b->d_pv, (size_t)c->L * n_pos * row * sizeof(float)));
        b->px_cap = (size_t)n_pos;
    }
    float* caches[2][2] = {{b->d_pk, c->d_kc}, {b->d_pv, c->d_vc}};
    for (auto& p : caches)
        for (int l = 0; l < c->L; ++l)
            HIPCHK(hipMemcpyAsync(p[0] + (size_t)l * n_pos * row, p[1] + (size_t)l * c->S * row, (size_t)n_pos * row * sizeof(float),
                                  hipMemcpyDeviceToDevice, c->stream));
    HIPCHK(hipStreamSynchronize(c->stream));
    b->P = n_pos;
    return LLMK_OK;
}

int llmk_prefix_attach(llmk_batch* b, int slot) {
    if (!b || slot < 0 || slot >= b->n_slots) return LLMK_E_ARG;
    if (b->P < 1) return LLMK_E_STATE;
    llmk_ctx* c = b->ctx;
    HIPCHK(hipSetDevice(c->cfg.device));
    const size_t slot_rows = (size_t)b->seq_len * c->KV;
    for (float* base : {b->d_kc, b->d_vc})
        for (int l = 0; l < c->L; ++l)
            HIPCHK(hipMemsetAsync(base + ((size_t)l * b->n_slots + slot) * slot_rows, 0, slot_rows * sizeof(float), c->stream));
    if (b->d_hist) HIPCHK(hipMemsetAsync(b->d_hist + (size_t)slot * b->seq_len, 0, (size_t)b->seq_len * sizeof(int), c->stream));
    HIPCHK(prefix_first(b, slot, b->P));
    HIPCHK(hipStreamSynchronize(c->stream));
    return LLMK_OK;
}

int llmk_prefix_len(llmk_batch* b) {
    if (!b) return -LLMK_E_ARG;
    return b->P;
}

int llmk_batch_forward(llmk_batch* b, int n, const int* slots, const int* tokens, const int* pos, float* logits_out, int* argmax_out) {
    if (!b || (!logits_out && !argmax_out) || !bd_rows_ok(b, n, slots, tokens, pos, 1)) return LLMK_E_ARG;
    llmk_ctx* c = b->ctx;
    ScPlan sp;
    int rc = bd_ready(b, &sp, n);
    if (rc) return rc;
    HIPCHK(bd_upload_rows(b, n, slots, tokens, pos));
    HIPCHK(bd_pass(b, n, *std::max_element(pos, pos + n), logits_out != nullptr, sp));
    HIPCHK(hipMemcpyAsync(b->h_out, b->d_out, (size_t)2 * n * sizeof(float), hipMemcpyDeviceToHost, c->stream));
    HIPCHK(bd_fetch_flag(c));
    HIPCHK(hipStreamSynchronize(c->stream));
    if (pf_flagged(c)) {
        static bool told = false;
        return pf_redo(c, "llmk_batch_forward", &told, [&] { return llmk_batch_forward(b, n, slots, tokens, pos, logits_out, argmax_out); });
    }
    const int* ids = reinterpret_cast<const int*>(b->h_out + n);
    for (int i = 0; i < n; ++i)
        if (ids[i] < 1 || ids[i] > c->V) return LLMK_E_NONFINITE;
    if (argmax_out) memcpy(argmax_out, ids, (size_t)n * sizeof(int));
    if (logits_out) HIPCHK(hipMemcpy(logits_out, b->d_logits, (size_t)n * c->V * sizeof(float), hipMemcpyDeviceToHost));
    return LLMK_OK;
}

static int rows_pen_setup(llmk_batch* b) {
    if (b->d_hist && b->d_pen_cnt && b->d_pen && b->h_pen) return LLMK_OK;
    llmk_ctx* c = b->ctx;
    HIPCHK(hipSetDevice(c->cfg.device));
    const size_t hist = (size_t)b->n_slots * b->seq_len * sizeof(int), cnt = (size_t)b->n_slots * c->V * sizeof(int);
    const size_t pen = (size_t)LLMK_MAX_BATCH * sizeof(llmk_penalty_params);
    if (!b->d_hist) {
        HIPCHK(dev_alloc(&b->d_hist, hist));
        HIPCHK(hipMemsetAsync(b->d_hist, 0, hist, c->stream));
    }
    if (!b->d_pen_cnt) {
        HIPCHK(dev_alloc(&b->d_pen_cnt, cnt));
        HIPCHK(hipMemsetAsync(b->d_pen_cnt, 0, cnt, c->stream));
    }
    if (!b->d_pen) {
        HIPCHK(dev_alloc(&b->d_pen, pen));
        HIPCHK(hipMemsetAsync(b->d_pen, 0, pen, c->stream));
    }
    if (!b->h_pen) {
        HIPCHK(hipHostMalloc(&b->h_pen, pen, hipHostMallocDefault));
        memset(b->h_pen, 0, pen);
    }
    HIPCHK(hipStreamSynchronize(c->stream));
    return LLMK_OK;
}
static int rows_lp_setup(llmk_batch* b, size_t nrec, bool raw) {
    llmk_ctx* c = b->ctx;
    HIPCHK(hipSetDevice(c->cfg.device));
    if (b->lp_cap < nrec) {
        HIPCHK(hipStreamSynchronize(c->stream));
        if (b->d_lp) { hipFree(b->d_lp); b->d_lp = nullptr; }
        if (b->h_lp) { hipHostFree(b->h_lp); b->h_lp = nullptr; }
        b->lp_cap = 0;
        HIPCHK(dev_alloc(&b->d_lp, nrec * sizeof(llmk_logprob_record)));
        HIPCHK(hipHostMalloc(&b->h_lp, nrec * sizeof(llmk_logprob_record), hipHostMallocDefault));
        b->lp_cap = nrec;
    }
    if (!b->d_lp_top) HIPCHK(dev_alloc(&b->d_lp_top, sizeof(unsigned)));
    if (!b->h_lp_top) HIPCHK(hipHostMalloc(&b->h_lp_top, sizeof(unsigned), hipHostMallocDefault));
    if (raw && !b->d_raw) HIPCHK(dev_alloc(&b->d_raw, (size_t)b->n_slots * c->V * sizeof(float)));
    return LLMK_OK;
}
static int rows_request(llmk_batch* b, int n, const llmk_sampler* samplers, const llmk_penalties* penalties, const llmk_logprobs* lp, size_t nrec,
                        bool* pen_on) {
    llmk_ctx* c = b->ctx;
// ... 61 lines not shown
                       const llmk_sampler* samplers, const llmk_penalties* penalties, const llmk_logprobs* lp, int* ids_out) {
    if (!b || !ids_out || steps < 1 || !bd_rows_ok(b, n, slots, tokens, pos0, steps)) return LLMK_E_ARG;
    llmk_ctx* c = b->ctx;
    const size_t nids = (size_t)n * steps;
    bool pen = false;
    int rc = rows_request(b, n, samplers, penalties, lp, nids, &pen);
    if (rc) return rc;
    ScPlan sp;
    if ((rc = bd_ready(b, &sp, n)) != LLMK_OK) return rc;
    if (b->ids_cap < nids) {
        if (b->d_ids) { hipFree(b->d_ids); b->d_ids = nullptr; b->ids_cap = 0; }
        HIPCHK(dev_alloc(&b->d_ids, nids * sizeof(int)));
        b->ids_cap = nids;
    }
    HIPCHK(bd_upload_rows(b, n, slots, tokens, pos0));
    HIPCHK(rows_upload_words(b, n, samplers != nullptr, pen, lp != nullptr));
    HIPCHK(hipMemsetAsync(b->d_err, 0, sizeof(unsigned), c->stream));
    const int max_pos0 = *std::max_element(pos0, pos0 + n);
    for (int s = 0; s < steps; ++s) {
        HIPCHK(bd_pass(b, n, max_pos0 + s, samplers != nullptr || lp != nullptr, sp, s));
        const int* picked = reinterpret_cast<const int*>(b->d_out + n);
        HIPCHK(rows_enqueue(b, n, samplers != nullptr, pen, true, lp != nullptr, steps, s, &picked));
        hipLaunchKernelGGL(bd_advance_kernel, dim3(1), dim3(LLMK_MAX_BATCH), 0, c->stream, picked, n, c->V, s, steps, b->d_ids, b->d_tok, b->d_rows, b->d_err);
        HIPCHK(hipGetLastError());
    }
    if (lp) HIPCHK(hipMemcpyAsync(b->h_lp, b->d_lp, nids * sizeof(llmk_logprob_record), hipMemcpyDeviceToHost, c->stream));
    HIPCHK(hipMemcpyAsync(b->h_err, b->d_err, sizeof(unsigned), hipMemcpyDeviceToHost, c->stream));
    HIPCHK(bd_fetch_flag(c));
    HIPCHK(hipStreamSynchronize(c->stream));
    if (pf_flagged(c)) {
        static bool told = false;
        return pf_redo(c, who, &told, [&] { return rows_decode(b, who, n, slots, tokens, pos0, steps, samplers, penalties, lp, ids_out); });
    }
    HIPCHK(hipMemcpy(ids_out, b->d_ids, nids * sizeof(int), hipMemcpyDeviceToHost));
    if (*b->h_err) return LLMK_E_NONFINITE;
    if (lp) rows_deliver(b, lp, nids);
    return LLMK_OK;
}

int llmk_batch_decode(llmk_batch* b, int n, const int* slots, const int* tokens, const int* pos0, int steps, const llmk_sampler* samplers, int* ids_out) {
    return rows_decode(b, "llmk_batch_decode", n, slots, tokens, pos0, steps, samplers, nullptr, nullptr, ids_out);
}
int llmk_rows_decode(llmk_batch* b, int n, const int* slots, const int* tokens, const int* pos0, int steps, const llmk_sampler* samplers,
                     const llmk_penalties* penalties, const llmk_logprobs* logprobs, int* ids_out) {
    return rows_decode(b, "llmk_rows_decode", n, slots, tokens, pos0, steps, samplers, penalties, logprobs, ids_out);
}

int llmk_rows_sample_logits(llmk_batch* b, int n, const int* slots, const int* pos, const float* logits, const llmk_sampler* samplers,
                            const llmk_penalties* penalties, const llmk_logprobs* logprobs, int* tokens_out, int* kept_out, float* tau_out,
                            float* adjusted_out) {
    if (!b || !logits || !samplers || !tokens_out || !bd_rows_ok(b, n, slots, nullptr, pos, 1, false)) return LLMK_E_ARG;
    llmk_ctx* c = b->ctx;
    int rc = check_ready(c);
    if (rc) return rc;
    HIPCHK(hipSetDevice(c->cfg.device));
    bool pen = false;
    if ((rc = rows_request(b, n, samplers, penalties, logprobs, (size_t)n, &pen)) != LLMK_OK) return rc;
    const size_t nv = (size_t)n * c->V * sizeof(float);
    std::vector<unsigned> out2((size_t)2 * n);
    HIPCHK(bd_upload_rows(b, n, slots, nullptr, pos));
    HIPCHK(rows_upload_words(b, n, true, pen, logprobs != nullptr));
    HIPCHK(hipMemcpyAsync(b->d_logits, logits, nv, hipMemcpyHostToDevice, c->stream));
    const int* picked = nullptr;
    HIPCHK(rows_enqueue(b, n, true, pen, false, logprobs != nullptr, 1, 0, &picked));
    HIPCHK(hipMemcpyAsync(tokens_out, picked, (size_t)n * sizeof(int), hipMemcpyDeviceToHost, c->stream));
    HIPCHK(hipMemcpyAsync(out2.data(), b->d_out2, out2.size() * sizeof(unsigned), hipMemcpyDeviceToHost, c->stream));
    if (adjusted_out) HIPCHK(hipMemcpyAsync(adjusted_out, b->d_logits, nv, hipMemcpyDeviceToHost, c->stream));
    if (logprobs) HIPCHK(hipMemcpyAsync(b->h_lp, b->d_lp, (size_t)n * sizeof(llmk_logprob_record), hipMemcpyDeviceToHost, c->stream));
    HIPCHK(hipStreamSynchronize(c->stream));
    for (int i = 0; i < n; ++i) {
        if (kept_out) kept_out[i] = (int)out2[2 * i];
        if (tau_out) memcpy(tau_out + i, &out2[2 * i + 1], sizeof(float));
    }
    for (int i = 0; i < n; ++i)
        if (tokens_out[i] < 1 || tokens_out[i] > c->V) return LLMK_E_NONFINITE;
    if (logprobs) rows_deliver(b, logprobs, (size_t)n);
    return LLMK_OK;
}

int llmk_rows_set_history(llmk_batch* b, int slot, const int* tokens, int n, int pos0) {
    if (!b || !tokens || slot < 0 || slot >= b->n_slots || n < 1 || pos0 < 1 || pos0 + n - 1 > b->seq_len) return LLMK_E_ARG;
    for (int i = 0; i < n; ++i)
        if (tokens[i] < 0 || tokens[i] > b->ctx->V) return LLMK_E_ARG;
    const int rc = rows_pen_setup(b);
    if (rc) return rc;
    hipStream_t st = b->ctx->stream;
    HIPCHK(hipMemcpyAsync(b->d_hist + (size_t)slot * b->seq_len + (pos0 - 1), tokens, (size_t)n * sizeof(int), hipMemcpyHostToDevice, st));
    HIPCHK(hipStreamSynchronize(st));
    return LLMK_OK;
}
int llmk_rows_get_history(llmk_batch* b, int slot, int* tokens_out, int n, int pos0) {
    if (!b || !tokens_out || slot < 0 || slot >= b->n_slots || n < 1 || pos0 < 1 || pos0 + n - 1 > b->seq_len) return LLMK_E_ARG;
    const int rc = rows_pen_setup(b);
    if (rc) return rc;
    hipStream_t st = b->ctx->stream;
    HIPCHK(hipMemcpyAsync(tokens_out, b->d_hist + (size_t)slot * b->seq_len + (pos0 - 1), (size_t)n * sizeof(int), hipMemcpyDeviceToHost, st));
    HIPCHK(hipStreamSynchronize(st));
    return LLMK_OK;
}

int llmk_batch_time(llmk_batch* b, int n, int pos, int iters, float* avg_ms) {
    if (!b || !avg_ms || n < 1 || n > b->n_slots || pos < 1 || pos > b->seq_len || iters < 1) return LLMK_E_ARG;
    for (int i = 0; i < n && b->n_attached > 0; ++i)
        if (pos <= b->h_first[i]) return LLMK_E_ARG;
    llmk_ctx* c = b->ctx;
    ScPlan sp;
    int rc = bd_ready(b, &sp, n);
    if (rc) return rc;
    int slots[LLMK_MAX_BATCH], tokens[LLMK_MAX_BATCH], posv[LLMK_MAX_BATCH];
    for (int i = 0; i < n; ++i) { slots[i] = i; tokens[i] = 1; posv[i] = pos; }
    HIPCHK(bd_upload_rows(b, n, slots, tokens, posv));
    HIPCHK(bd_pass(b, n, pos, false, sp));
    HIPCHK(hipStreamSynchronize(c->stream));
    hipEvent_t e0 = nullptr, e1 = nullptr;
    HIPCHK(hipEventCreate(&e0));
    hipError_t pe = hipEventCreate(&e1);
    if (pe == hipSuccess) pe = hipEventRecord(e0, c->stream);
    for (int k = 0; k < iters && pe == hipSuccess; ++k) pe = bd_pass(b, n, pos, false, sp);
    if (pe == hipSuccess) pe = hipEventRecord(e1, c->stream);
    if (pe == hipSuccess) pe = hipStreamSynchronize(c->stream);
    float ms = 0.f;
    if (pe == hipSuccess) pe = hipEventElapsedTime(&ms, e0, e1);
    hipEventDestroy(e0);
    if (e1) hipEventDestroy(e1);
    HIPCHK(hipMemsetAsync(c->pf_flag, 0, sizeof(unsigned), c->stream));
    HIPCHK(hipStreamSynchronize(c->stream));
    if (pe != hipSuccess) return LLMK_E_HIP + (int)pe;
    *avg_ms = ms / (float)iters;
    return LLMK_OK;
}

int llmk_reset(llmk_ctx* c) {
    if (!c) return LLMK_E_ARG;
    HIPCHK(hipSetDevice(c->cfg.device));
    const size_t kvn = (size_t)c->L * c->S * c->KVl * sizeof(float);
    HIPCHK(hipMemsetAsync(c->d_kc, 0, kvn, c->stream));
    HIPCHK(hipMemsetAsync(c->d_vc, 0, kvn, c->stream));
    HIPCHK(hipMemsetAsync(&c->dev_words()->err, 0, sizeof(unsigned), c->stream));
    HIPCHK(tk_qsc_clear(c, c->stream));
    if (c->d_hist) {
        HIPCHK(hipMemsetAsync(c->d_hist, 0, (size_t)c->S * sizeof(int), c->stream));
        HIPCHK(hipMemsetAsync(c->d_pen_cnt, 0, (size_t)c->V * sizeof(int), c->stream));
    }
    HIPCHK(hipStreamSynchronize(c->stream));
    c->host_words()->err = 0;
    c->h_next->err = 0;
    for (int i = 0; i < 5; ++i) c->times[i] = 0.f;
    return LLMK_OK;
}

int llmk_timings(llmk_ctx* c, float ms[5]) {
    if (!c || !ms) return LLMK_E_ARG;
    for (int i = 0; i < 5; ++i) ms[i] = c->times[i];
    return LLMK_OK;
}

int llmk_time_kernel(llmk_ctx* c, int kernel, int iters, float* avg_ms, double* bytes_per_launch) {
    int rc = check_ready(c);
    if (rc) return rc;
    if (kernel < 0 || kernel > 12 || iters <= 0 || !avg_ms) return LLMK_E_ARG;
    if (kernel == 6 && !c->use_tk) return LLMK_E_ARG;
    HIPCHK(hipSetDevice(c->cfg.device));
    if (kernel == 11) {
        if (c->h_tokpos[1] < 1) { c->h_tokpos[0] = 0; c->h_tokpos[1] = 1; }
        HIPCHK(hipMemcpyAsync(c->d_tokpos, c->h_tokpos, 4 * sizeof(int), hipMemcpyHostToDevice, c->stream));
        hipGraph_t g = nullptr;
        hipGraphExec_t ge = nullptr;
        HIPCHK(hipStreamBeginCapture(c->stream, hipStreamCaptureModeThreadLocal));
        hipError_t e = hipSuccess;
        for (int l = 0; l < c->L && e == hipSuccess; ++l) {
            e = launch_qkv(c, l);
            if (e == hipSuccess) e = launch_attn(c, l);
            if (e == hipSuccess) e = launch_wo(c, l);
            if (e == hipSuccess) e = launch_w13(c, l);
            if (e == hipSuccess) e = launch_w2(c, l);
        }
        const hipError_t e2 = hipStreamEndCapture(c->stream, &g);
        if (e != hipSuccess || e2 != hipSuccess) { if (g) hipGraphDestroy(g); return LLMK_E_HIP + (int)(e != hipSuccess ? e : e2); }
        e = hipGraphInstantiate(&ge, g, nullptr, nullptr, 0);
        hipGraphDestroy(g);
        HIPCHK(e);
        for (int i = 0; i < 3 && e == hipSuccess; ++i) e = hipGraphLaunch(ge, c->stream);
        if (e == hipSuccess) e = hipEventRecord(c->ev[6], c->stream);
        for (int i = 0; i < iters && e == hipSuccess; ++i) e = hipGraphLaunch(ge, c->stream);
        if (e == hipSuccess) e = hipEventRecord(c->ev[7], c->stream);
        if (e == hipSuccess) e = hipEventSynchronize(c->ev[7]);
        float ms = 0.f;
        if (e == hipSuccess) e = hipEventElapsedTime(&ms, c->ev[6], c->ev[7]);
        hipGraphExecDestroy(ge);
        HIPCHK(e);
        *avg_ms = ms / (float)iters / (float)c->L;
        if (bytes_per_launch) {
            double b = 0;
            for (int m : {LLMK_WQKV, LLMK_WO, LLMK_W13, LLMK_W2}) b += (double)c->desc[m].rows * (double)row_bytes_for(c->t[m].type, c->desc[m].K);
            *bytes_per_launch = b;
        }
        return LLMK_OK;
    }
    ScPlan sp{0, 0, 0};
    if (kernel >= 7) {
        const int pf_step = PF_KSTEP;
        if (c->tp_size != 1 || c->E % pf_step || c->H % pf_step) return LLMK_E_ARG;
        rc = pf_setup(c, true);
        if (rc) return rc;
        if (kernel == 12) {
            sp = sc_plan(c);
            if (sp.R == 0) return LLMK_E_ARG;
        }
        HIPCHK(hipMemsetAsync(c->pf[0].Xs, 0x3c, (size_t)PF_TMAX * c->E * sizeof(float), c->stream));
        HIPCHK(hipMemsetAsync(c->pf[0].HB, 0x3c, (size_t)PF_TMAX * c->H * sizeof(float), c->stream));
    }
    if (c->h_tokpos[1] < 1) { c->h_tokpos[0] = 0; c->h_tokpos[1] = 1; }
    HIPCHK(hipMemcpyAsync(c->d_tokpos, c->h_tokpos, 4 * sizeof(int), hipMemcpyHostToDevice, c->stream));
    auto one = [&](int i) -> hipError_t {
        int l = i % c->L;
#ifdef LLMK_PF_TRACE
        if (getenv("LLMK_PF_ONE_LAYER")) l = 0;
#endif
        if (kernel == 6) {
            hipLaunchKernelGGL(bump_serial_kernel, dim3(1), dim3(1), 0, c->stream, c->d_tokpos);
            return launch_token_kernel(c);
        }
        if (kernel == 12) {
            PfEpiArgs e;
            const DevTensor& ct = c->t[LLMK_WCLS];
            for (int k = 0; k < sp.nchunks; ++k) {
                const int r0 = k * sp.R;
                HIPRET(pf_gemm(c, c->pf[0], (const char*)ct.data + (size_t)r0 * ct.row_bytes, (int)ct.row_bytes, c->pf[0].Xs, std::min(sp.R, c->V - r0), c->E,
                               PF_TMAX, &e, ct.type));
            }
            return hipSuccess;
        }
        if (kernel >= 7) {
            PfEpiArgs e;
            const int tid = kernel == 7 ? LLMK_W13 : kernel == 8 ? LLMK_WQKV : kernel == 9 ? LLMK_WO : LLMK_W2;
            const int rows = kernel == 7 ? 2 * c->H : kernel == 8 ? c->E + 2 * c->KV : c->E;
            const char* w = (const char*)c->t[tid].data + (size_t)l * rows * c->t[tid].row_bytes;
            const float* X = kernel == 10 ? c->pf[0].HB : c->pf[0].Xs;
            const int K = kernel == 10 ? c->H : c->E;
            return pf_gemm(c, c->pf[0], w, (int)c->t[tid].row_bytes, X, rows, K, PF_TMAX, &e);
        }
        switch (kernel) {
            case 0: return launch_qkv(c, l);
            case 1: return launch_attn(c, l);
            case 2: return launch_wo(c, l);
            case 3: return launch_w13(c, l);
            case 4: return launch_w2(c, l);
            default: return launch_cls(c);
        }
    };
    for (int i = 0; i < 3; ++i) HIPCHK(one(i));
    HIPCHK(hipEventRecord(c->ev[6], c->stream));
    for (int i = 0; i < iters; ++i) HIPCHK(one(i + 3));
    HIPCHK(hipEventRecord(c->ev[7], c->stream));
    HIPCHK(hipEventSynchronize(c->ev[7]));
    float ms = 0.f;
    HIPCHK(hipEventElapsedTime(&ms, c->ev[6], c->ev[7]));
    *avg_ms = ms / (float)iters;
    if (kernel == 6) c->h_tokpos[2] += iters + 3;
    if (bytes_per_launch) {
        const int tids[13] = {LLMK_WQKV, -1, LLMK_WO, LLMK_W13, LLMK_W2, LLMK_WCLS, -1, LLMK_W13, LLMK_WQKV, LLMK_WO, LLMK_W2, -1, LLMK_WCLS};
        double b = 0;
        if (kernel == 6) {
            double w = 0;
            const int mats[5] = {LLMK_WQKV, LLMK_WO, LLMK_W13, LLMK_W2, LLMK_WCLS};
            for (int m : mats) w += (double)c->desc[m].rows * (c->desc[m].layered ? c->L : 1) * (double)row_bytes_for(c->t[m].type, c->desc[m].K);
            b = w + (2.0 * c->L + 1) * c->E * 4 + c->E * 4 + 2.0 * c->L * c->KV * 4.0 * c->h_tokpos[1] +
                2.0 * c->L * c->KV * 4 + c->V * 4.0;
        } else if (kernel == 1) {
            b = 2.0 * c->KV * 4.0 * c->h_tokpos[1];
        } else {
            const TensorDesc& d = c->desc[tids[kernel]];
            const int type = c->t[tids[kernel]].type;
            b = (double)d.rows * (double)(kernel == 12 && type == LLMK_TYPE_Q6_K ? dev_row_bytes(type, d.K) : row_bytes_for(type, d.K));
        }
        *bytes_per_launch = b;
    }
    return LLMK_OK;
}

int llmk_cls_form(llmk_ctx* c, int rows) {
    if (!c || rows < 1 || rows > LLMK_MAX_BATCH) return -LLMK_E_ARG;
    int rc = check_ready(c);
    if (rc) return -rc;
    if (!pf_shape_ok(c)) return LLMK_CLS_NONE;
    auto setup = [&]() -> int {
        HIPCHK(hipSetDevice(c->cfg.device));
        return pf_setup(c, true);
    };
    if ((rc = setup()) != LLMK_OK) return -rc;
    if (sc_plan(c, rows).R > 0) return LLMK_CLS_GEMM;
    return c->t[LLMK_WCLS].type == LLMK_TYPE_Q6_K ? LLMK_CLS_ROWS : LLMK_CLS_NONE;
}

int llmk_peek(llmk_ctx* c, int which, int layer, int pos, float* out, int n) {
    if (!c || !out || n <= 0) return LLMK_E_ARG;
    HIPCHK(hipSetDevice(c->cfg.device));
    const float* src = nullptr;
    int len = 0;
    switch (which) {
        case 0: src = c->d_x; len = c->E; break;
        case 1: src = c->d_q; len = c->Eq; break;
        case 2: src = c->d_xb; len = c->Eq; break;
        case 3: src = c->d_hb; len = c->Hl; break;
        case 4:
        case 5:
            if (layer < 0 || layer >= c->L || pos < 1 || pos > c->S) return LLMK_E_ARG;
            src = (which == 4 ? c->d_kc : c->d_vc) + ((size_t)layer * c->S + (pos - 1)) * c->KVl;
            len = c->KVl;
            break;
#ifdef LLMK_PF_TRACE
        case 7: src = c->pf[0].HB; len = PF_TMAX * c->H; break;
#endif
        case 8: {
            size_t ng;
            src = reinterpret_cast<const float*>(tk_qsc_records(c, &ng));
            if (!src) return LLMK_E_ARG;
            len = (int)(2 * ng);
            break;
        }
        case 6:
            if (!c->d_trace) return LLMK_E_ARG;
            src = (const float*)c->d_trace; len = TK_NCU * TK_TRACE_N * 2;
            break;
        default: return LLMK_E_ARG;
    }
    if (n > len) return LLMK_E_ARG;
    HIPCHK(hipStreamSynchronize(c->stream));
    HIPCHK(hipMemcpy(out, src, (size_t)n * sizeof(float), hipMemcpyDeviceToHost));
    return LLMK_OK;
}

int llmk_tp_unique_id(char id_out[128]) {
    if (!id_out) return LLMK_E_ARG;
    static_assert(sizeof(ncclUniqueId) == 128, "ncclUniqueId is 128 bytes");
    ncclUniqueId id;
    if (ncclGetUniqueId(&id) != ncclSuccess) return LLMK_E_COMM;
    memcpy(id_out, &id, sizeof(id));
    return LLMK_OK;
}

int llmk_tp_init_comm(llmk_ctx* c, const char id_in[128]) {
    if (!c || !id_in || c->comm) return LLMK_E_ARG;
    if (c->p2p) return LLMK_E_STATE;
    HIPCHK(hipSetDevice(c->cfg.device));
    ncclUniqueId id;
    memcpy(&id, id_in, sizeof(id));
    if (ncclCommInitRank(&c->comm, c->tp_size, id, c->tp_rank) != ncclSuccess) { c->comm = nullptr; return LLMK_E_COMM; }
    return LLMK_OK;
}

static int tp_inbox_alloc(llmk_ctx* c) {
    if (c->d_inbox) return LLMK_OK;
    if (c->tp_size < 2 || c->tp_size > TP_MAX_RANKS) return LLMK_E_ARG;
    HIPCHK(hipSetDevice(c->cfg.device));
    const size_t bytes = tp_inbox_granules(c->tp_size, c->E, c->V) * sizeof(unsigned long long);
    HIPCHK(hipExtMallocWithFlags((void**)&c->d_inbox, bytes, hipDeviceMallocFinegrained));
    HIPCHK(hipMemset(c->d_inbox, 0, bytes));
    HIPCHK(dev_alloc(&c->d_tp_bad, sizeof(unsigned)));
    HIPCHK(hipDeviceSynchronize());
    c->peers.inbox[c->tp_rank] = c->d_inbox;
    int khz = 0;
    if (hipDeviceGetAttribute(&khz, hipDeviceAttributeWallClockRate, c->cfg.device) != hipSuccess || khz <= 0) khz = 100000;
    const long long ms = getenv("LLMK_TP_TIMEOUT_MS") ? atoll(getenv("LLMK_TP_TIMEOUT_MS")) : 20000;
    c->peers.timeout_ticks = (unsigned long long)(ms > 0 ? ms : 20000) * (unsigned long long)khz;
    return LLMK_OK;
}

int llmk_tp_p2p_handle(llmk_ctx* c, char handle_out[64]) {
    if (!c || !handle_out) return LLMK_E_ARG;
    int rc = tp_inbox_alloc(c);
    if (rc) return rc;
    static_assert(sizeof(hipIpcMemHandle_t) == 64, "hipIpcMemHandle_t is 64 bytes");
    hipIpcMemHandle_t h;
    HIPCHK(hipIpcGetMemHandle(&h, c->d_inbox));
    memcpy(handle_out, &h, sizeof(h));
    return LLMK_OK;
}

int llmk_tp_p2p_connect(llmk_ctx* c, const char* handles) {
    if (!c || !handles || c->p2p) return LLMK_E_ARG;
    int rc = tp_inbox_alloc(c);
    if (rc) return rc;
    for (int r = 0; r < c->tp_size; ++r) {
        if (r == c->tp_rank) continue;
        hipIpcMemHandle_t h;
        memcpy(&h, handles + (size_t)r * 64, sizeof(h));
        void* p = nullptr;
        HIPCHK(hipIpcOpenMemHandle(&p, h, hipIpcMemLazyEnablePeerAccess));
        c->ipc_mapped[r] = p;
        c->peers.inbox[r] = (unsigned long long*)p;
    }
    c->p2p = true;
    return LLMK_OK;
}

int llmk_tp_p2p_connect_local(llmk_ctx* c, llmk_ctx* const* ranks) {
    if (!c || !ranks || c->p2p) return LLMK_E_ARG;
    int rc = tp_inbox_alloc(c);
    if (rc) return rc;
    for (int r = 0; r < c->tp_size; ++r) {
        if (r == c->tp_rank) continue;
        llmk_ctx* o = ranks[r];
        if (!o || o->tp_size != c->tp_size || o->tp_rank != r || o->E != c->E || o->V != c->V) return LLMK_E_ARG;
        rc = tp_inbox_alloc(o);
        if (rc) return rc;
        HIPCHK(hipSetDevice(c->cfg.device));
        if (o->cfg.device != c->cfg.device) {
            const hipError_t e = hipDeviceEnablePeerAccess(o->cfg.device, 0);
            if (e != hipSuccess && e != hipErrorPeerAccessAlreadyEnabled) return LLMK_E_HIP + (int)e;
            (void)hipGetLastError();
        }
        c->peers.inbox[r] = o->d_inbox;
    }
    c->p2p = true;
    return LLMK_OK;
}

__global__ void tp_selftest_fill_kernel(float* part, float* x, float* logits, int E, int V, int me, int P, int it) {
    const int i = blockIdx.x * blockDim.x + threadIdx.x;
    if (i < E) { part[i] = (float)((i * 7 + me * 13 + it) % 1021); x[i] = 0.f; }
    if (i < V) logits[i] = (i / (V / P) == me) ? (float)((i * 3 + it) % 4093) : -1.f;
}
__global__ void tp_selftest_check_kernel(const float* x, const float* logits, int E, int V, int P, int it, unsigned* bad) {
    const int i = blockIdx.x * blockDim.x + threadIdx.x;
    if (i < E) {
        float want = 0.f;
        for (int r = 0; r < P; ++r) want += (float)((i * 7 + r * 13 + it) % 1021);
        if (x[i] != 2.f * want) atomicAdd(bad, 1u);
    }
    if (i < V && logits[i] != (float)((i * 3 + it) % 4093)) atomicAdd(bad, 1u);
}
static int tp_selftest_run(llmk_ctx* c, int iters, unsigned jseed) {
    if (!c || iters < 1) return LLMK_E_ARG;
    if (!c->p2p) return LLMK_E_COMM;
    HIPCHK(hipSetDevice(c->cfg.device));
    unsigned* d_bad = c->d_tp_bad;
    if (!d_bad) return LLMK_E_COMM;
    HIPCHK(hipMemsetAsync(d_bad, 0, sizeof(unsigned), c->stream));
    const int n = std::max(c->E, c->V);
    int rc = LLMK_OK;
    hipError_t e0 = hipMemcpyAsync(c->d_tokpos, c->h_tokpos, 4 * sizeof(int), hipMemcpyHostToDevice, c->stream);
    if (e0 == hipSuccess) e0 = hipStreamSynchronize(c->stream);
    if (e0 != hipSuccess) rc = LLMK_E_HIP + (int)e0;
    for (int it = 0; it < iters && rc == LLMK_OK; ++it) {
        const unsigned js = jseed ? (jseed + (unsigned)it * 2654435761u) | 1u : 0u;
        hipLaunchKernelGGL(bump_serial_kernel, dim3(1), dim3(1), 0, c->stream, c->d_tokpos);
        hipError_t e = hipGetLastError();
        if (e == hipSuccess) {
            hipLaunchKernelGGL(tp_selftest_fill_kernel, dim3((n + 255) / 256), dim3(256), 0, c->stream, c->d_part, c->d_x, c->d_logits, c->E,
                               c->V, c->tp_rank, c->tp_size, it);
            e = launch_tp_allreduce_add(c, 0, js);
        }
        if (e == hipSuccess) e = launch_tp_allreduce_add(c, 1, js);
        if (e == hipSuccess) e = launch_tp_allgather(c, js);
        if (e == hipSuccess) {
            hipLaunchKernelGGL(tp_selftest_check_kernel, dim3((n + 255) / 256), dim3(256), 0, c->stream, c->d_x, c->d_logits, c->E, c->V,
                               c->tp_size, it, d_bad);
            e = hipGetLastError();
        }
        if (e != hipSuccess) rc = LLMK_E_HIP + (int)e;
        if (jseed && (it & 63) == 63 && rc == LLMK_OK) { e = hipStreamSynchronize(c->stream); if (e != hipSuccess) rc = LLMK_E_HIP + (int)e; }
    }
    c->h_tokpos[2] += iters;
    unsigned bad = 0, err = 0;
    if (rc == LLMK_OK) {
        hipError_t e = hipStreamSynchronize(c->stream);
        if (e == hipSuccess) e = hipMemcpy(&bad, d_bad, sizeof(bad), hipMemcpyDeviceToHost);
        if (e == hipSuccess) e = hipMemcpy(&err, &c->dev_words()->err, sizeof(err), hipMemcpyDeviceToHost);
        if (e != hipSuccess) rc = LLMK_E_HIP + (int)e;
        else if (err) rc = LLMK_E_TIMEOUT;
        else if (bad) rc = LLMK_E_COMM;
    }
    hipMemsetAsync(c->d_x, 0, (size_t)c->E * sizeof(float), c->stream);
    hipMemsetAsync(c->d_logits, 0, (size_t)c->V * sizeof(float) + offsetof(TkDevWords, cand), c->stream);
    hipStreamSynchronize(c->stream);
    if (rc != LLMK_OK) {
        char what[160];
        fprintf(stderr, "llmk: rank %d of %d: the peer-memory collectives failed their %s (%s, %u mismatches, %s)\n",
                c->tp_rank, c->tp_size, jseed ? "stress run" : "self-test",
                rc == LLMK_E_TIMEOUT ? "a peer's granules never arrived" : rc == LLMK_E_COMM ? "wrong sums" : "HIP error", bad,
                tp_describe_err(c, err, what, sizeof(what)));
    }
    return rc;
}
int llmk_tp_p2p_selftest(llmk_ctx* c, int iters) { return tp_selftest_run(c, iters, 0u); }
int llmk_tp_p2p_stress(llmk_ctx* c, int iters, unsigned seed) { return tp_selftest_run(c, iters, seed | 1u); }

int llmk_tp_p2p_disable(llmk_ctx* c) {
    if (!c) return LLMK_E_ARG;
    HIPCHK(hipSetDevice(c->cfg.device));
    HIPCHK(hipStreamSynchronize(c->stream));
    c->p2p = false;
    drop_graphs(c);
    return LLMK_OK;
}

int llmk_tp_begin(llmk_ctx* c, int token, int pos) {
    int rc = check_ready(c);
    if (rc) return rc;
    if (token < 1 || token > c->V || pos < 1 || pos > c->S) return LLMK_E_ARG;
    HIPCHK(hipSetDevice(c->cfg.device));
    c->h_tokpos[0] = token - 1;
    c->h_tokpos[1] = pos;
    c->h_tokpos[2] += 1;
    HIPCHK(hipMemcpyAsync(c->d_tokpos, c->h_tokpos, 4 * sizeof(int), hipMemcpyHostToDevice, c->stream));
    HIPCHK(launch_embed(c));
    HIPCHK(hipStreamSynchronize(c->stream));
    return LLMK_OK;
}

int llmk_tp_segment(llmk_ctx* c, int seg, int layer) {
    int rc = check_ready(c);
    if (rc) return rc;
    if (seg < 0 || seg > 2 || layer < 0 || layer >= c->L) return LLMK_E_ARG;
    HIPCHK(hipSetDevice(c->cfg.device));
    if (seg == 0) {
        if (layer > 0) HIPCHK(launch_add_partial(c));
        HIPCHK(launch_qkv(c, layer));
        HIPCHK(launch_attn(c, layer));
        HIPCHK(launch_wo(c, layer));
    } else if (seg == 1) {
        HIPCHK(launch_add_partial(c));
        HIPCHK(launch_w13(c, layer));
        HIPCHK(launch_w2(c, layer));
    } else {
        HIPCHK(launch_add_partial(c));
        HIPCHK(launch_cls(c));
    }
    HIPCHK(hipStreamSynchronize(c->stream));
    return LLMK_OK;
}

int llmk_tp_read_partial(llmk_ctx* c, float* out) {
    if (!c || !out) return LLMK_E_ARG;
    HIPCHK(hipSetDevice(c->cfg.device));
    HIPCHK(hipMemcpy(out, c->d_part, (size_t)c->E * sizeof(float), hipMemcpyDeviceToHost));
    return LLMK_OK;
}
int llmk_tp_write_partial(llmk_ctx* c, const float* in) {
    if (!c || !in) return LLMK_E_ARG;
    HIPCHK(hipSetDevice(c->cfg.device));
    HIPCHK(hipMemcpy(c->d_part, in, (size_t)c->E * sizeof(float), hipMemcpyHostToDevice));
    return LLMK_OK;
}
int llmk_tp_read_logits(llmk_ctx* c, float* out_slice) {
    if (!c || !out_slice) return LLMK_E_ARG;
    HIPCHK(hipSetDevice(c->cfg.device));
    HIPCHK(hipMemcpy(out_slice, c->d_logits + (size_t)c->tp_rank * c->Vl, (size_t)c->Vl * sizeof(float), hipMemcpyDeviceToHost));
    return LLMK_OK;
}

__global__ void checksum_kernel(const unsigned* __restrict__ w, size_t nwords, unsigned long long* out) {
    unsigned long long t = 0;
    for (size_t i = (size_t)blockIdx.x * blockDim.x + threadIdx.x; i < nwords; i += (size_t)gridDim.x * blockDim.x) t += w[i];
    for (int o = 32; o > 0; o >>= 1) t += __shfl_xor(t, o, 64);
    if ((threadIdx.x & 63) == 0) atomicAdd(out, t);
}
int llmk_tensor_checksum(llmk_ctx* c, int tid, unsigned long long* out) {
    if (!c || !out || tid < 0 || tid >= LLMK_N_TENSORS) return LLMK_E_ARG;
    const TensorDesc& d = c->desc[tid];
    const DevTensor& t = c->t[tid];
    if (!t.data) return LLMK_E_STATE;
    HIPCHK(hipSetDevice(c->cfg.device));
    const size_t nwords = (size_t)d.rows * (d.layered ? c->L : 1) * t.row_bytes / 4;
    unsigned long long* d_out = nullptr;
    HIPCHK(dev_alloc(&d_out, sizeof(*d_out)));
    hipError_t e = hipMemsetAsync(d_out, 0, sizeof(*d_out), c->stream);
    if (e == hipSuccess) {
        hipLaunchKernelGGL(checksum_kernel, dim3(1024), dim3(256), 0, c->stream, (const unsigned*)t.data, nwords, d_out);
        e = hipGetLastError();
    }
    if (e == hipSuccess) e = hipMemcpyAsync(out, d_out, sizeof(*d_out), hipMemcpyDeviceToHost, c->stream);
    if (e == hipSuccess) e = hipStreamSynchronize(c->stream);
    hipFree(d_out);
    return e == hipSuccess ? LLMK_OK : LLMK_E_HIP + (int)e;
}

int llmk_tk_shapes(char* buf, size_t n) {
    if (!buf || n == 0) return LLMK_E_ARG;
    static const char* tn[] = {"f32", "f16", "q4_0"};
    size_t o = 0;
    buf[0] = 0;
    for (int i = 0; i < TK_NSHAPES; ++i) {
        const TkEntry& e = tk_table[i];
        char one[96];
        const int k = snprintf(one, sizeof(one), "%s%d,%d,%d,%d,%d,%s%s", i ? ";" : "", e.E, e.H, e.NH, e.NKV, e.V, tn[e.WT], e.CLS != e.WT ? "+q6_K" : "");
        if (o + (size_t)k + 1 > n) return LLMK_E_SIZE;
        memcpy(buf + o, one, (size_t)k + 1);
        o += (size_t)k;
    }
    return LLMK_OK;
}

int llmk_path(llmk_ctx* c) {
    if (!c) return -LLMK_E_ARG;
    if (c->p2p) return LLMK_PATH_TP_P2P;
    if (c->comm) return LLMK_PATH_TP_RCCL;
    if (c->tp_size > 1) return LLMK_PATH_TP_UNCONNECTED;
    return c->use_tk ? LLMK_PATH_TOKEN_KERNEL : LLMK_PATH_MULTI_KERNEL;
}

int llmk_tp_ranks_seen(llmk_ctx* c) {
    if (!c) return -LLMK_E_ARG;
    if (c->comm) {
        int n = 0;
        if (ncclCommCount(c->comm, &n) != ncclSuccess) return -LLMK_E_COMM;
        return n;
    }
    if (c->p2p) {
        int n = 0;
        for (int r = 0; r < c->tp_size; ++r) n += c->peers.inbox[r] != nullptr;
        return n;
    }
    return 1;
}

int llmk_destroy(llmk_ctx* c) {
    if (!c) return LLMK_E_ARG;
    if (c->n_batches > 0) return LLMK_E_STATE;
    hipSetDevice(c->cfg.device);
    if (c->stream) hipStreamSynchronize(c->stream);
    if (c->comm) ncclCommDestroy(c->comm);
    for (int r = 0; r < TP_MAX_RANKS; ++r)
        if (c->ipc_mapped[r]) hipIpcCloseMemHandle(c->ipc_mapped[r]);
    if (c->d_inbox) hipFree(c->d_inbox);
    if (c->d_tp_bad) hipFree(c->d_tp_bad);
    drop_graphs(c);
    for (int i = 0; i < LLMK_N_TENSORS; ++i) {
        if (c->t[i].data && !c->t[i].alias) hipFree(c->t[i].data);
    }
    pf_teardown(c);
    sc_teardown(c);
    void* dev[] = {c->d_kc, c->d_vc, c->d_x, c->d_q, c->d_xb, c->d_hb, c->d_logits, c->d_rope, c->d_tokpos, c->d_next,
                   c->d_gran, c->d_zeros, c->d_trace, c->d_part, c->d_hist, c->d_pen_cnt, c->d_pen, c->d_lp, c->d_lp_raw};
    for (void* p : dev)
        if (p) hipFree(p);
    for (int b = 0; b < 2; ++b) {
        if (c->up_stage[b]) hipHostFree(c->up_stage[b]);
        if (c->up_tmp[b]) hipFree(c->up_tmp[b]);
        if (c->up_done[b]) hipEventDestroy(c->up_done[b]);
    }
    if (c->up_acc) hipFree(c->up_acc);
    for (int i = 0; i < LLMK_N_TENSORS; ++i)
        if (c->q16[i]) hipFree(c->q16[i]);
    if (c->h_tokpos) hipHostFree(c->h_tokpos);
    if (c->h_logits) hipHostFree(c->h_logits);
    if (c->h_next) hipHostFree(c->h_next);
    if (c->h_samp) hipHostFree(c->h_samp);
    if (c->h_filt) hipHostFree(c->h_filt);
    if (c->h_pen) hipHostFree(c->h_pen);
    if (c->h_lp) hipHostFree(c->h_lp);
    if (c->h_lp_top) hipHostFree(c->h_lp_top);
    for (int i = 0; i < 8; ++i)
        if (c->ev[i]) hipEventDestroy(c->ev[i]);
    if (c->stream) hipStreamDestroy(c->stream);
    delete c;
    return LLMK_OK;
}

}
```

### llm.f90_amd/llmk.py

```python
from __future__ import annotations

import ctypes as C
import os
import subprocess

import numpy as np

_HERE = os.path.dirname(os.path.abspath(__file__))
LIB_PATH = os.environ.get("LLMK_LIB") or os.path.join(_HERE, "csrc", "libllmk.so")

TENSOR_IDS = {
    "token_embedding_table": 0, "rms_att_weight": 1, "rms_ffn_weight": 2, "wqkv": 3, "wo": 4, "w13": 5, "w2": 6,
    "rms_final_weight": 7, "wcls": 8,
}
FLAG_NO_GRAPH, FLAG_TIMINGS, FLAG_MULTI_KERNEL = 1, 2, 4
SYMBOLS = ["llmk_create", "llmk_create_tp", "llmk_tp_unique_id", "llmk_tp_init_comm", "llmk_tp_p2p_handle", "llmk_tp_p2p_connect",
           "llmk_tp_p2p_connect_local", "llmk_tp_p2p_selftest", "llmk_tp_p2p_stress", "llmk_tp_p2p_disable", "llmk_tp_begin", "llmk_tp_segment",
           "llmk_tp_read_partial", "llmk_tp_write_partial", "llmk_tp_read_logits", "llmk_upload", "llmk_upload_rows",
           "llmk_set_rope_freqs", "llmk_set_tensor_type", "llmk_set_rms_eps", "llmk_forward", "llmk_prefill", "llmk_forward_greedy", "llmk_decode_greedy",
           "llmk_forward_sample", "llmk_decode_sample", "llmk_forward_sample_ex", "llmk_decode_sample_ex", "llmk_sample_logits", "llmk_set_history", "llmk_get_history",
           "llmk_forward_sample_pen", "llmk_decode_sample_pen", "llmk_sample_logits_pen", "llmk_forward_sample_lp", "llmk_decode_sample_lp",
           "llmk_logprob_logits", "llmk_score", "llmk_batch_create", "llmk_batch_destroy", "llmk_batch_fork", "llmk_batch_forward",
           "llmk_batch_decode", "llmk_batch_time", "llmk_rows_set_history", "llmk_rows_get_history", "llmk_rows_decode",
           "llmk_rows_sample_logits", "llmk_prefix_set", "llmk_prefix_attach", "llmk_prefix_len", "llmk_reset", "llmk_timings",
           "llmk_time_kernel", "llmk_cls_form", "llmk_peek", "llmk_tensor_checksum", "llmk_path", "llmk_tk_shapes", "llmk_tp_ranks_seen", "llmk_destroy", "llmk_strerror", "llmk_version"]
PATH_NAMES = {0: "multi-kernel (5 launches per layer)", 1: "persistent whole-token kernel",
              2: "tensor-parallel rank: 6 launches per layer + one-shot peer-memory exchanges",
              3: "tensor-parallel rank: eager launches + RCCL collectives", 4: "tensor-parallel rank, collectives not connected"}


TOKEN_FN = C.CFUNCTYPE(None, C.c_int, C.c_int, C.c_void_p)


class LlmkError(RuntimeError):
    def __init__(self, code, msg):
        super().__init__(f"llmk error {code}: {msg}")
        self.code = code


class Config(C.Structure):
    _fields_ = [(n, C.c_int32) for n in ("emb_dim", "hidden_dim", "n_layers", "n_heads", "n_kv_heads", "vocab_size",
                                         "seq_len", "weight_type", "device", "flags")]


class Sampler(C.Structure):
    _fields_ = [("temperature", C.c_float), ("top_k", C.c_int32), ("top_p", C.c_float), ("min_p", C.c_float), ("seed", C.c_uint64)]


def sampler(temperature: float, seed: int, top_k: int = 0, top_p: float = 1.0, min_p: float = 0.0) -> Sampler:
    return Sampler(temperature, top_k, top_p, min_p, seed & 0xFFFFFFFFFFFFFFFF)


MAX_LOGIT_BIAS = 256
MAX_BATCH = 128
CLS_NONE, CLS_GEMM, CLS_ROWS = 0, 1, 2


class LogitBias(C.Structure):
    _fields_ = [("token", C.c_int32), ("bias", C.c_float)]


class Penalties(C.Structure):
    _fields_ = [("last_n", C.c_int32), ("repeat", C.c_float), ("frequency", C.c_float), ("presence", C.c_float),
                ("bias", C.POINTER(LogitBias)), ("n_bias", C.c_int32)]


def penalties(last_n: int = 0, repeat: float = 1.0, frequency: float = 0.0, presence: float = 0.0, bias=()) -> Penalties:
    items = list(bias.items()) if isinstance(bias, dict) else list(bias)
    arr = (LogitBias * max(1, len(items)))(*[LogitBias(int(t), float(b)) for t, b in items])
    pn = Penalties(last_n, repeat, frequency, presence, C.cast(arr, C.POINTER(LogitBias)), len(items))
    pn._entries = arr
    return pn


MAX_TOP_LOGPROBS = 20


class Logprobs(C.Structure):
    _fields_ = [("top_n", C.c_int32), ("token_logprob", C.POINTER(C.c_float)), ("top_tokens", C.POINTER(C.c_int32)),
                ("top_logprobs", C.POINTER(C.c_float))]


def logprobs(n: int, top_n: int, want_token: bool = True) -> Logprobs:
    lp = Logprobs(top_n, None, None, None)
    lp.token = np.zeros(n, np.float32) if want_token else None
    lp.tokens = np.zeros((n, max(top_n, 0)), np.int32)
    lp.values = np.zeros((n, max(top_n, 0)), np.float32)
    if want_token:
        lp.token_logprob = lp.token.ctypes.data_as(C.POINTER(C.c_float))
    if top_n > 0:
        lp.top_tokens = lp.tokens.ctypes.data_as(C.POINTER(C.c_int32))
        lp.top_logprobs = lp.values.ctypes.data_as(C.POINTER(C.c_float))
    return lp


def _request(temperature, seed, top_k, top_p, min_p, *pen):
    return C.byref(sampler(temperature, seed, top_k, top_p, min_p)), C.byref(penalties(*pen))


def build_lib(force: bool = False) -> str:
    subprocess.run(["make", "-s", "-C", _HERE, "lib"] + (["-B"] if force else []), check=True)
    return LIB_PATH


_lib = None


def lib():
    global _lib
    if _lib is None:
        if not os.path.exists(LIB_PATH):
            raise FileNotFoundError(f"{LIB_PATH} not built (run `make -C llm.f90_amd lib`); there is no CPU fallback")
        L = C.CDLL(LIB_PATH)
        vp, ci, cf = C.c_void_p, C.c_int, C.POINTER(C.c_float)
        L.llmk_create.argtypes = [C.POINTER(Config), C.POINTER(vp)]
        L.llmk_create_tp.argtypes = [C.POINTER(Config), ci, ci, C.POINTER(vp)]
        L.llmk_tp_unique_id.argtypes = [C.c_char_p]
        L.llmk_tp_init_comm.argtypes = [vp, C.c_char_p]
        L.llmk_tp_p2p_handle.argtypes = [vp, C.c_char_p]
        L.llmk_tp_p2p_connect.argtypes = [vp, C.c_char_p]
        L.llmk_tp_p2p_connect_local.argtypes = [vp, C.POINTER(vp)]
        L.llmk_tp_p2p_selftest.argtypes = [vp, ci]
        L.llmk_tp_p2p_stress.argtypes = [vp, ci, C.c_uint]
        L.llmk_tp_p2p_disable.argtypes = [vp]
        L.llmk_tensor_checksum.argtypes = [vp, ci, C.POINTER(C.c_ulonglong)]
        L.llmk_tp_begin.argtypes = [vp, ci, ci]
        L.llmk_tp_segment.argtypes = [vp, ci, ci]
        L.llmk_tp_read_partial.argtypes = [vp, cf]
        L.llmk_tp_write_partial.argtypes = [vp, cf]
        L.llmk_tp_read_logits.argtypes = [vp, cf]
        L.llmk_upload.argtypes = [vp, ci, vp, C.c_size_t, ci]
        L.llmk_upload_rows.argtypes = [vp, ci, ci, ci, ci, vp, C.c_size_t, ci]
        L.llmk_set_rope_freqs.argtypes = [vp, cf, ci]
        L.llmk_set_tensor_type.argtypes = [vp, ci, ci]
        L.llmk_set_rms_eps.argtypes = [vp, C.c_float]
        L.llmk_forward.argtypes = [vp, ci, ci, cf]
        L.llmk_prefill.argtypes = [vp, C.POINTER(ci), ci, ci, cf]
        L.llmk_forward_greedy.argtypes = [vp, ci, ci, C.POINTER(ci)]
        L.llmk_decode_greedy.argtypes = [vp, ci, ci, ci, C.POINTER(ci), vp, vp]
        if hasattr(L, "llmk_forward_sample"):
            L.llmk_forward_sample.argtypes = [vp, ci, ci, C.c_float, C.c_uint64, C.POINTER(ci)]
            L.llmk_decode_sample.argtypes = [vp, ci, ci, ci, C.c_float, C.c_uint64, C.POINTER(ci), vp, vp]
        if hasattr(L, "llmk_sample_logits"):
            L.llmk_forward_sample_ex.argtypes = [vp, ci, ci, C.POINTER(Sampler), C.POINTER(ci)]
            L.llmk_decode_sample_ex.argtypes = [vp, ci, ci, ci, C.POINTER(Sampler), C.POINTER(ci), vp, vp]
            L.llmk_sample_logits.argtypes = [vp, cf, ci, C.POINTER(Sampler), C.POINTER(ci), C.POINTER(ci), cf]
        if hasattr(L, "llmk_sample_logits_pen"):
            L.llmk_set_history.argtypes = [vp, C.POINTER(ci), ci, ci]
            L.llmk_get_history.argtypes = [vp, C.POINTER(ci), ci, ci]
            L.llmk_forward_sample_pen.argtypes = [vp, ci, ci, C.POINTER(Sampler), C.POINTER(Penalties), C.POINTER(ci)]
            L.llmk_decode_sample_pen.argtypes = [vp, ci, ci, ci, C.POINTER(Sampler), C.POINTER(Penalties), C.POINTER(ci), vp, vp]
            L.llmk_sample_logits_pen.argtypes = [vp, cf, ci, C.POINTER(Sampler), C.POINTER(Penalties), C.POINTER(ci), C.POINTER(ci), cf, cf]
        if hasattr(L, "llmk_logprob_logits"):
            L.llmk_forward_sample_lp.argtypes = [vp, ci, ci, C.POINTER(Sampler), C.POINTER(Penalties), C.POINTER(Logprobs), C.POINTER(ci)]
            L.llmk_decode_sample_lp.argtypes = [vp, ci, ci, ci, C.POINTER(Sampler), C.POINTER(Penalties), C.POINTER(Logprobs), C.POINTER(ci), vp, vp]
            L.llmk_logprob_logits.argtypes = [vp, cf, ci, ci, cf, C.POINTER(C.c_int32), cf]
        if hasattr(L, "llmk_score"):
            L.llmk_score.argtypes = [vp, C.POINTER(ci), ci, ci, C.POINTER(ci), cf, C.POINTER(ci), cf]
        if hasattr(L, "llmk_batch_create"):
            L.llmk_batch_create.argtypes = [vp, ci, ci, C.POINTER(vp)]
            L.llmk_batch_destroy.argtypes = [vp]
            L.llmk_batch_fork.argtypes = [vp, ci, ci]
            L.llmk_batch_forward.argtypes = [vp, ci, C.POINTER(ci), C.POINTER(ci), C.POINTER(ci), cf, C.POINTER(ci)]
            L.llmk_batch_decode.argtypes = [vp, ci, C.POINTER(ci), C.POINTER(ci), C.POINTER(ci), ci, C.POINTER(Sampler), C.POINTER(ci)]
            L.llmk_batch_time.argtypes = [vp, ci, ci, ci, cf]
        if hasattr(L, "llmk_rows_decode"):
            pi = C.POINTER(ci)
            L.llmk_rows_set_history.argtypes = [vp, ci, pi, ci, ci]
            L.llmk_rows_get_history.argtypes = [vp, ci, pi, ci, ci]
            L.llmk_rows_decode.argtypes = [vp, ci, pi, pi, pi, ci, C.POINTER(Sampler), C.POINTER(Penalties), C.POINTER(Logprobs), pi]
            L.llmk_rows_sample_logits.argtypes = [vp, ci, pi, pi, cf, C.POINTER(Sampler), C.POINTER(Penalties), C.POINTER(Logprobs), pi, pi, cf, cf]
        if hasattr(L, "llmk_prefix_set"):
            L.llmk_prefix_set.argtypes = [vp, ci]
            L.llmk_prefix_attach.argtypes = [vp, ci]
            L.llmk_prefix_len.argtypes = [vp]
        L.llmk_reset.argtypes = [vp]
        L.llmk_timings.argtypes = [vp, cf]
        L.llmk_time_kernel.argtypes = [vp, ci, ci, cf, C.POINTER(C.c_double)]
        if hasattr(L, "llmk_cls_form"):
            L.llmk_cls_form.argtypes = [vp, ci]
        L.llmk_peek.argtypes = [vp, ci, ci, ci, cf, ci]
        L.llmk_destroy.argtypes = [vp]
        L.llmk_path.argtypes = [vp]
        if hasattr(L, "llmk_tk_shapes"):
            L.llmk_tk_shapes.argtypes = [C.c_char_p, C.c_size_t]
        L.llmk_tp_ranks_seen.argtypes = [vp]
        L.llmk_strerror.argtypes = [ci]
        L.llmk_strerror.restype = C.c_char_p
        L.llmk_version.argtypes = []
        for s in SYMBOLS:
            if s != "llmk_strerror" and (hasattr(L, s) or not os.environ.get("LLMK_LIB")):
                getattr(L, s).restype = ci
        _lib = L
    return _lib


def _ck(rc):
    if rc != 0:
        raise LlmkError(rc, lib().llmk_strerror(rc).decode())


def tk_shapes():
    buf = C.create_string_buffer(8192)
    _ck(lib().llmk_tk_shapes(buf, len(buf)))
    out = []
    for item in buf.value.decode().split(";"):
        f = item.split(",")
        out.append(tuple(int(x) for x in f[:5]) + (f[5],))
    return out


class Llmk:

    def __init__(self, fw, device: int = 0, flags: int = 0, seq_len: int | None = None, tp_rank: int = 0,
                 tp_size: int = 1):
        s = fw.shape
        self.shape = s
        self.V = s.vocab_size
        self.tp_rank, self.tp_size = tp_rank, tp_size
        cfg = Config(s.emb_dim, s.hidden_dim, s.n_layers, s.n_heads, s.n_kv_heads, s.vocab_size,
                     seq_len or s.seq_len, fw.ggml_type, device, flags)
        self._h = C.c_void_p()
        _ck(lib().llmk_create_tp(C.byref(cfg), tp_rank, tp_size, C.byref(self._h)))
        cls_type = getattr(fw, "cls_type", fw.ggml_type)
        if cls_type != fw.ggml_type:
            _ck(lib().llmk_set_tensor_type(self._h, TENSOR_IDS["wcls"], cls_type))
        for name, tid in TENSOR_IDS.items():
            a = np.ascontiguousarray(getattr(fw, name))
            is_mat = name in ("wqkv", "wo", "w13", "w2", "wcls")
            _ck(lib().llmk_upload(self._h, tid, a.ctypes.data, a.nbytes,
                                  (cls_type if name == "wcls" else fw.ggml_type) if is_mat else 0))
        self._finish_init()

    def _finish_init(self):
        hs = self.shape.head_size
        fr = np.float32(1.0) / np.power(np.float32(10000.0), (np.arange(1, hs, 2, dtype=np.float32) / np.float32(hs)),
                                        dtype=np.float32)
        self.set_rope_freqs(fr)
        self._logits = np.empty(self.V, np.float32)

    @classmethod
    def create_empty(cls, shape, ggml_type: int, device: int = 0, flags: int = 0, tp_rank: int = 0, tp_size: int = 1,
                     seq_len: int | None = None) -> "Llmk":
        m = cls.__new__(cls)
        m.shape, m.V, m.tp_rank, m.tp_size = shape, shape.vocab_size, tp_rank, tp_size
        cfg = Config(shape.emb_dim, shape.hidden_dim, shape.n_layers, shape.n_heads, shape.n_kv_heads, shape.vocab_size,
                     seq_len or shape.seq_len, ggml_type, device, flags)
        m._h = C.c_void_p()
        _ck(lib().llmk_create_tp(C.byref(cfg), tp_rank, tp_size, C.byref(m._h)))
        m._finish_init()
        return m

    def upload_rows(self, name: str, layer: int, row0: int, arr, ggml_type: int):
        arr = np.ascontiguousarray(arr)
        _ck(lib().llmk_upload_rows(self._h, TENSOR_IDS[name], layer, row0, arr.shape[0] if arr.ndim > 1 else 1, arr.ctypes.data,
                                   arr.nbytes, ggml_type))

    def set_rope_freqs(self, fr):
        fr = np.ascontiguousarray(fr, np.float32)
        _ck(lib().llmk_set_rope_freqs(self._h, fr.ctypes.data_as(C.POINTER(C.c_float)), len(fr)))

    def set_tensor_type(self, name: str, ggml_type: int):
        _ck(lib().llmk_set_tensor_type(self._h, TENSOR_IDS[name], ggml_type))

    def set_rms_eps(self, eps: float):
        _ck(lib().llmk_set_rms_eps(self._h, eps))

    def forward(self, token: int, pos: int) -> np.ndarray:
        _ck(lib().llmk_forward(self._h, token, pos, self._logits.ctypes.data_as(C.POINTER(C.c_float))))
        return self._logits.copy()

    def forward_raw(self, token: int, pos: int) -> int:
        return lib().llmk_forward(self._h, token, pos, self._logits.ctypes.data_as(C.POINTER(C.c_float)))

    def prefill(self, tokens, pos0: int = 1) -> np.ndarray:
        t = np.ascontiguousarray(tokens, np.int32)
        _ck(lib().llmk_prefill(self._h, t.ctypes.data_as(C.POINTER(C.c_int)), len(t), pos0,
                               self._logits.ctypes.data_as(C.POINTER(C.c_float))))
        return self._logits.copy()

    def score(self, tokens, pos0: int = 1, targets=None, want_argmax: bool = False, want_logits: bool = False, want_logprob: bool = True):
        t = np.ascontiguousarray(tokens, np.int32)
        n = len(t)
        ip, fp = C.POINTER(C.c_int), C.POINTER(C.c_float)
        tg = lp = am = lg = None
        if want_logprob:
            tg = np.ascontiguousarray(np.append(t[1:], 0) if targets is None else targets, np.int32)
            if len(tg) != n:
                raise ValueError("one target per token")
            lp = np.empty(n, np.float32)
        if want_argmax:
            am = np.empty(n, np.int32)
        if want_logits:
            lg = np.empty((n, self.V), np.float32)
        _ck(lib().llmk_score(self._h, t.ctypes.data_as(ip), n, pos0, tg.ctypes.data_as(ip) if tg is not None else None,
                             lp.ctypes.data_as(fp) if lp is not None else None, am.ctypes.data_as(ip) if am is not None else None,
                             lg.ctypes.data_as(fp) if lg is not None else None))
        out = [a for a in (lp, am, lg) if a is not None]
        return out[0] if len(out) == 1 else tuple(out)

    def forward_greedy(self, token: int, pos: int) -> int:
        nxt = C.c_int(0)
        _ck(lib().llmk_forward_greedy(self._h, token, pos, C.byref(nxt)))
        return nxt.value

    def _decode(self, fn, token: int, pos0: int, n: int, on_token, *request) -> np.ndarray:
        ids = np.zeros(n, np.int32)
        cb = TOKEN_FN(on_token) if on_token else None
        _ck(fn(self._h, token, pos0, n, *request, ids.ctypes.data_as(C.POINTER(C.c_int)), C.cast(cb, C.c_void_p) if cb else None, None))
        return ids

    def decode_greedy(self, token: int, pos0: int, n: int, on_token=None) -> np.ndarray:
        return self._decode(lib().llmk_decode_greedy, token, pos0, n, on_token)

    def forward_sample(self, token: int, pos: int, temperature: float, seed: int) -> int:
        nxt = C.c_int(0)
        _ck(lib().llmk_forward_sample(self._h, token, pos, temperature, seed & 0xFFFFFFFFFFFFFFFF, C.byref(nxt)))
        return nxt.value

    def decode_sample(self, token: int, pos0: int, n: int, temperature: float, seed: int, on_token=None) -> np.ndarray:
        return self._decode(lib().llmk_decode_sample, token, pos0, n, on_token, temperature, seed & 0xFFFFFFFFFFFFFFFF)

    def forward_sample_ex(self, token: int, pos: int, temperature: float, seed: int, top_k: int = 0, top_p: float = 1.0,
                          min_p: float = 0.0) -> int:
        nxt = C.c_int(0)
        sp, _ = _request(temperature, seed, top_k, top_p, min_p)
        _ck(lib().llmk_forward_sample_ex(self._h, token, pos, sp, C.byref(nxt)))
        return nxt.value

    def decode_sample_ex(self, token: int, pos0: int, n: int, temperature: float, seed: int, top_k: int = 0, top_p: float = 1.0,
                         min_p: float = 0.0, on_token=None) -> np.ndarray:
        sp, _ = _request(temperature, seed, top_k, top_p, min_p)
        return self._decode(lib().llmk_decode_sample_ex, token, pos0, n, on_token, sp)

    def sample_logits(self, logits, pos: int, temperature: float, seed: int, top_k: int = 0, top_p: float = 1.0, min_p: float = 0.0):
        lg = np.ascontiguousarray(logits, np.float32)
        if lg.shape != (self.V,):
            raise ValueError("one logit per vocabulary row")
        tok, kept, tau = C.c_int(0), C.c_int(0), C.c_float(0)
        sp, _ = _request(temperature, seed, top_k, top_p, min_p)
        _ck(lib().llmk_sample_logits(self._h, lg.ctypes.data_as(C.POINTER(C.c_float)), pos, sp, C.byref(tok), C.byref(kept), C.byref(tau)))
        return tok.value, kept.value, tau.value

    def set_history(self, tokens, pos0: int = 1):
        t = np.ascontiguousarray(tokens, np.int32)
        _ck(lib().llmk_set_history(self._h, t.ctypes.data_as(C.POINTER(C.c_int)), len(t), pos0))

    def get_history(self, n: int, pos0: int = 1) -> np.ndarray:
        out = np.zeros(n, np.int32)
        _ck(lib().llmk_get_history(self._h, out.ctypes.data_as(C.POINTER(C.c_int)), n, pos0))
        return out

    def forward_sample_pen(self, token: int, pos: int, temperature: float, seed: int, top_k: int = 0, top_p: float = 1.0,
                           min_p: float = 0.0, last_n: int = 0, repeat: float = 1.0, frequency: float = 0.0, presence: float = 0.0,
                           bias=()) -> int:
        nxt = C.c_int(0)
        sp, pn = _request(temperature, seed, top_k, top_p, min_p, last_n, repeat, frequency, presence, bias)
# ... 301 lines not shown
```

Baseline: 1364 tokens/s.

## Speculatively launch next decode step using device greedy id in llmk_forward

Adds a forward-ahead mode to llmk_forward. Once the host has been seen picking the argmax of the previous logits, it launches the next token pass early, feeding it the greedy id the GPU computed, and double-buffers logits in pinned host memory. The next call checks the published id against the real token: a hit returns the already-computed logits, and a miss syncs, falls back to a normal pass and backs off exponentially. The aim is to hide host-side memcpy, argmax and launch latency behind GPU compute, at the cost of added state, settle calls on every other API entry point, and wasted work on mispredictions.

```diff
diff --git a/include/llmk.h b/include/llmk.h
--- a/include/llmk.h
+++ b/include/llmk.h
@@ -87,6 +87,8 @@
 int llmk_set_rope_freqs(llmk_ctx *ctx, const float *freqs, int n);
 
 int llmk_forward(llmk_ctx *ctx, int token, int pos, float *logits_out);
+
+int llmk_forward_ahead_stats(llmk_ctx *ctx, int out[4]);
 
 int llmk_prefill(llmk_ctx* ctx, const int* tokens, int n, int pos0, float* logits_out);
 
diff --git a/llm.f90_amd/csrc/forward_ahead.h b/llm.f90_amd/csrc/forward_ahead.h
--- /dev/null
+++ b/llm.f90_amd/csrc/forward_ahead.h
@@ -0,0 +1,72 @@
+#ifndef LLMK_FORWARD_AHEAD_H
+#define LLMK_FORWARD_AHEAD_H
+
+namespace llmk {
+
+inline int fa_first_max(const float* v, int n) {
+    float bv = -__builtin_inff();
+    int bi = -1;
+    for (int i = 0; i < n; ++i)
+        if (v[i] > bv) { bv = v[i]; bi = i; }
+    return bi;
+}
+
+struct ForwardAhead {
+    static constexpr int ARM_STREAK = 2;
+    static constexpr int BACKOFF_FIRST = 16;
+    static constexpr int BACKOFF_MAX = 1024;
+
+    bool armed = false;
+    int next = 0;
+    int last = 0;
+    int streak = 0;
+    int skip = 0;
+    int backoff = 0;
+    int launches = 0, hits = 0, misses = 0, scans = 0;
+
+    bool scan_due(int pos) {
+        if (armed || last == 0 || pos != last + 1) { streak = 0; return false; }
+        if (skip > 0) { --skip; return false; }
+        ++scans;
+        return true;
+    }
+    bool scanned(bool agree, int pos, int S) {
+        if (!agree) { disagree(); return false; }
+        if (++streak < ARM_STREAK || pos >= S) return false;
+        armed = true;
+        next = pos + 1;
+        ++launches;
+        return true;
+    }
+    bool expects(int pos) const { return armed && pos == next; }
+    bool hit(int S) {
+        ++hits;
+        if (next + 1 <= S) { ++next; ++launches; return true; }
+        armed = false;
+        streak = 0;
+        return false;
+    }
+    void miss() {
+        ++misses;
+        armed = false;
+        last = 0;
+        disagree();
+    }
+    void ran(int pos) { last = pos; }
+    void interrupt() {
+        armed = false;
+        last = 0;
+        streak = 0;
+    }
+
+private:
+    void disagree() {
+        streak = 0;
+        backoff = backoff == 0 ? BACKOFF_FIRST : backoff >= BACKOFF_MAX / 2 ? BACKOFF_MAX : 2 * backoff;
+        skip = backoff;
+    }
+};
+
+}
+
+#endif
diff --git a/llm.f90_amd/csrc/llmk.hip b/llm.f90_amd/csrc/llmk.hip
--- a/llm.f90_amd/csrc/llmk.hip
+++ b/llm.f90_amd/csrc/llmk.hip
@@ -4,6 +4,7 @@
 #include "prefill.h"
 #include "batch.h"
 #include "tp_p2p.h"
+#include "forward_ahead.h"
 
 #include <rccl/rccl.h>
 
@@ -164,6 +165,14 @@
     size_t sc_logits_cap = 0;
     bool sc_ready = false;
     int n_batches = 0;
+    bool fa_on = true;
+    ForwardAhead fa;
+    bool fa_inflight = false;
+    float* fa_buf[2] = {nullptr, nullptr};
+    float* fa_buf_dev[2] = {nullptr, nullptr};
+    const float* fa_logits = nullptr;
+    int fa_tok0 = 0, fa_pos = 0;
+    hipEvent_t fa_ev[2] = {nullptr, nullptr};
 };
 typedef llmk_ctx::PfLane PfLane;
 
@@ -395,7 +404,7 @@
         if (e_ != hipSuccess) return e_; \
     } while (0)
 
-struct TkGreedy { int gflags = 0, id_index = 0; };
+struct TkGreedy { int gflags = 0, id_index = 0; float* logits = nullptr; };
 template <class TK>
 hipError_t launch_token_kernel_t(llmk_ctx* c, bool direct, const TkGreedy& g) {
     TokenArgs a;
@@ -415,7 +424,7 @@
     a.pos_imm = c->h_tokpos[1];
     a.serial_imm = c->h_tokpos[2];
     a.g_qkv = c->d_gran;
-    a.logits = direct ? c->h_logits_dev : c->d_logits;
+    a.logits = g.logits ? g.logits : direct ? c->h_logits_dev : c->d_logits;
     a.err = &c->dev_words()->err;
     a.herr = (direct || g.gflags) ? &c->host_words_dev()->err : nullptr;
     a.zeros = c->d_zeros;
@@ -691,12 +700,17 @@
     return LLMK_OK;
 }
 
-int check_ready(llmk_ctx* c) {
-    if (!c) return LLMK_E_ARG;
+int tensors_ready(llmk_ctx* c) {
     for (int i = 0; i < LLMK_N_TENSORS; ++i)
         if (!c->t[i].uploaded) return LLMK_E_STATE;
     if (c->use_tk && tk_table[c->tk_shape - 1].q4 && c->q16_dirty) return q16_build(c);
     return LLMK_OK;
+}
+int spec_settle(llmk_ctx* c);
+int check_ready(llmk_ctx* c) {
+    if (!c) return LLMK_E_ARG;
+    const int rc = spec_settle(c);
+    return rc ? rc : tensors_ready(c);
 }
 
 constexpr int TK_RANGE_LIMIT = 4;
@@ -740,9 +754,27 @@
                   call, serial, call / 2u, (call & 1u) ? "w2" : "wo");
     return buf;
 }
+int spec_settle(llmk_ctx* c) {
+    c->fa.interrupt();
+    if (!c->fa_inflight) return LLMK_OK;
+    HIPCHK(hipSetDevice(c->cfg.device));
+    HIPCHK(hipStreamSynchronize(c->stream));
+    c->fa_inflight = false;
+    c->h_tokpos[0] = c->fa_tok0;
+    c->h_tokpos[1] = c->fa_pos;
+    unsigned err = 0;
+    HIPCHK(hipMemcpy(&err, &c->dev_words()->err, sizeof(unsigned), hipMemcpyDeviceToHost));
+    if (err == 0) return LLMK_OK;
+    return (err & 0x2000u) ? tk_clear_err(c) : tk_retire(c, err, c->fa_pos + 1);
+}
+
+int token_pass(llmk_ctx* c, int token, int pos, TailMode tail);
 int run_token_pass(llmk_ctx* c, int token, int pos, TailMode tail) {
-    int rc = check_ready(c);
-    if (rc) return rc;
+    const int rc = check_ready(c);
+    return rc ? rc : token_pass(c, token, pos, tail);
+}
+int token_pass(llmk_ctx* c, int token, int pos, TailMode tail) {
+    int rc;
     if (token < 1 || token > c->V || pos < 1 || pos > c->S) return LLMK_E_ARG;
     HIPCHK(hipSetDevice(c->cfg.device));
     c->h_tokpos[0] = token - 1;
@@ -1345,6 +1377,12 @@
     CK(hipHostMalloc(&c->h_logits, (size_t)V * sizeof(float) + sizeof(TkHostWords) + (size_t)S * sizeof(int), hipHostMallocMapped));
     CK(hipHostGetDevicePointer((void**)&c->h_logits_dev, c->h_logits, 0));
     c->tk_direct = !(getenv("LLMK_TK_DIRECT") && getenv("LLMK_TK_DIRECT")[0] == '0');
+    c->fa_on = !(getenv("LLMK_FORWARD_AHEAD") && getenv("LLMK_FORWARD_AHEAD")[0] == '0');
+    c->fa_buf[0] = c->h_logits;
+    c->fa_buf_dev[0] = c->h_logits_dev;
+    CK(hipHostMalloc(&c->fa_buf[1], (size_t)V * sizeof(float), hipHostMallocMapped));
+    CK(hipHostGetDevicePointer((void**)&c->fa_buf_dev[1], c->fa_buf[1], 0));
+    for (int i = 0; i < 2; ++i) CK(hipEventCreateWithFlags(&c->fa_ev[i], hipEventDisableTiming));
     CK(hipHostMalloc(&c->h_next, sizeof(TkNext), hipHostMallocDefault));
     CK(hipHostMalloc(&c->h_samp, sizeof(llmk_sample_params), hipHostMallocDefault));
     CK(hipHostMalloc(&c->h_filt, sizeof(llmk_filter_params), hipHostMallocDefault));
@@ -1595,6 +1633,7 @@
     if (ggml_type != t.type) return LLMK_E_TYPE;
     if (nbytes != (size_t)rows * row_bytes_for(ggml_type, g.K)) return LLMK_E_SIZE;
     HIPCHK(hipSetDevice(c->cfg.device));
+    { const int rc = spec_settle(c); if (rc) return rc; }
     if (c->tp_size > 1) return upload_rows_sharded(c, tid, layer, row_offset, rows, (const uint8_t*)host, ggml_type);
     const size_t pitch = row_bytes_for(ggml_type, g.K);
     return upload_block(c, tid, layer, row_offset, rows, (const uint8_t*)host, pitch, 0, pitch);
@@ -1625,6 +1664,7 @@
     const int kalign = ggml_type == LLMK_TYPE_Q6_K ? Q6K_WEIGHTS : ggml_type == LLMK_TYPE_Q4_0 ? 32 : ggml_type == LLMK_TYPE_F16 ? 8 : 4;
     if (d.K % kalign) return LLMK_E_SHAPE;
     HIPCHK(hipSetDevice(c->cfg.device));
+    { const int rc = spec_settle(c); if (rc) return rc; }
     HIPCHK(hipStreamSynchronize(c->stream));
     if (t.data) HIPCHK(hipFree(t.data));
     if (c->pf_ready) pf_teardown(c);
@@ -1654,6 +1694,7 @@
 int llmk_set_rms_eps(llmk_ctx* c, float eps) {
     if (!c || !(eps > 0.f) || !(eps < 1.f)) return LLMK_E_ARG;
     HIPCHK(hipSetDevice(c->cfg.device));
+    { const int rc = spec_settle(c); if (rc) return rc; }
     HIPCHK(hipStreamSynchronize(c->stream));
     c->eps = eps;
     drop_graphs(c);
@@ -1663,15 +1704,118 @@
 int llmk_set_rope_freqs(llmk_ctx* c, const float* freqs, int n) {
     if (!c || !freqs || n != c->hs / 2) return LLMK_E_ARG;
     HIPCHK(hipSetDevice(c->cfg.device));
+    { const int rc = spec_settle(c); if (rc) return rc; }
     HIPCHK(hipMemcpy(c->d_rope, freqs, (size_t)n * sizeof(float), hipMemcpyHostToDevice));
+    return LLMK_OK;
+}
+
+static bool fa_eligible(const llmk_ctx* c) {
+    if (!c->fa_on || !c->use_tk || !c->tk_direct || c->tp_size != 1 || c->comm || c->p2p) return false;
+    if ((c->cfg.flags & (LLMK_FLAG_TIMINGS | LLMK_FLAG_NO_GRAPH)) || tk_table[c->tk_shape - 1].q4) return false;
+    return !(TK_DEBUG && getenv("LLMK_TK_INJECT_TIMEOUT"));
+}
+static int fa_launch(llmk_ctx* c, int token, int pos, bool spec) {
+    if (!spec) c->h_tokpos[0] = token - 1;
+    c->h_tokpos[1] = pos;
+    c->h_tokpos[2] += 1;
+    TkGreedy g;
+    g.gflags = TKG_GREEDY | (spec ? TKG_CAND_IN | TKG_ID : 0);
+    g.id_index = pos - 2;
+    g.logits = c->fa_buf_dev[pos & 1];
+    if (spec) {
+        c->host_words()->ids()[pos - 2] = 0;
+        c->fa_inflight = true;
+    }
+    c->tk_short_grid = false;
+    HIPCHK(launch_token_kernel(c, true, g));
+    HIPCHK(hipEventRecord(c->fa_ev[pos & 1], c->stream));
+    return LLMK_OK;
+}
+static int fa_published_id(llmk_ctx* c, int slot, int* id) {
+    volatile int* ids = c->host_words()->ids();
+    while ((*id = ids[slot]) == 0) {
+        const hipError_t q = hipStreamQuery(c->stream);
+        if (q == hipSuccess) { *id = ids[slot]; break; }
+        if (q != hipErrorNotReady) return LLMK_E_HIP + (int)q;
+    }
+    return LLMK_OK;
+}
+static int fa_deliver(llmk_ctx* c, int token, int pos, bool more, float* logits_out) {
+    HIPCHK(more ? hipEventSynchronize(c->fa_ev[pos & 1]) : hipStreamSynchronize(c->stream));
+    if (!more) c->fa_inflight = false;
+    const unsigned err = c->host_words()->err;
+    if (err != 0) {
+        c->fa_inflight = true;
+        const int rc = spec_settle(c);
+        if (rc) return rc;
+        if (!(err & 0x2000u)) {
+            const int rc2 = token_pass(c, token, pos, TAIL_LOGITS);
+            if (rc2) return rc2;
+            memcpy(logits_out, c->h_logits, (size_t)c->V * sizeof(float));
+            return LLMK_OK;
+        }
+    }
+    c->tk_range_run = 0;
+    memcpy(logits_out, c->fa_buf[pos & 1], (size_t)c->V * sizeof(float));
+    if (err == 0) {
+        c->fa_logits = c->fa_buf[pos & 1];
+        c->fa.ran(pos);
+    }
+    c->fa_tok0 = token - 1;
+    c->fa_pos = pos;
     return LLMK_OK;
 }
 
 int llmk_forward(llmk_ctx* c, int token, int pos, float* logits_out) {
     if (!c || !logits_out) return LLMK_E_ARG;
-    int rc = run_token(c, token, pos, TAIL_LOGITS);
-    if (rc) return rc;
+    if (!fa_eligible(c)) {
+        int rc = run_token(c, token, pos, TAIL_LOGITS);
+        if (rc) return rc;
+        memcpy(logits_out, c->h_logits, (size_t)c->V * sizeof(float));
+        return LLMK_OK;
+    }
+    int rc = tensors_ready(c);
+    if (rc == LLMK_OK && (token < 1 || token > c->V || pos < 1 || pos > c->S)) rc = LLMK_E_ARG;
+    if (rc == LLMK_OK && hipSetDevice(c->cfg.device) != hipSuccess) rc = LLMK_E_HIP;
+    if (rc) { spec_settle(c); return rc; }
+    ForwardAhead& fa = c->fa;
+    if (fa.armed) {
+        int id = 0;
+        if (fa.expects(pos) && (rc = fa_published_id(c, pos - 2, &id)) != LLMK_OK) { spec_settle(c); return rc; }
+        if (id == token) {
+            const bool more = fa.hit(c->S);
+            if (more && (rc = fa_launch(c, 0, pos + 1, true)) != LLMK_OK) { spec_settle(c); return rc; }
+            if ((rc = fa_deliver(c, token, pos, more, logits_out)) != LLMK_OK) spec_settle(c);
+            return rc;
+        }
+        fa.miss();
+        if ((rc = spec_settle(c)) != LLMK_OK) return rc;
+    } else if (fa.scan_due(pos) && fa.scanned(fa_first_max(c->fa_logits, c->V) + 1 == token, pos, c->S)) {
+        TkDevWords* dw = c->dev_words();
+        hipError_t e = c->samp_dev.push(llmk_sample_params{}, [&] { return hipMemsetAsync(&dw->samp, 0, sizeof(llmk_sample_params), c->stream); });
+        if (e != hipSuccess) { spec_settle(c); return LLMK_E_HIP + (int)e; }
+        c->host_words()->err = 0;
+        if ((rc = fa_launch(c, token, pos, false)) == LLMK_OK) rc = fa_launch(c, 0, pos + 1, true);
+        if (rc == LLMK_OK) rc = fa_deliver(c, token, pos, true, logits_out);
+        if (rc) spec_settle(c);
+        return rc;
+    }
+    rc = token_pass(c, token, pos, TAIL_LOGITS);
+    if (rc) { fa.interrupt(); return rc; }
     memcpy(logits_out, c->h_logits, (size_t)c->V * sizeof(float));
+    c->fa_logits = c->h_logits;
+    c->fa_tok0 = token - 1;
+    c->fa_pos = pos;
+    if (fa_eligible(c)) fa.ran(pos);
+    return LLMK_OK;
+}
+
+int llmk_forward_ahead_stats(llmk_ctx* c, int out[4]) {
+    if (!c || !out) return LLMK_E_ARG;
+    out[0] = c->fa.launches;
+    out[1] = c->fa.hits;
+    out[2] = c->fa.misses;
+    out[3] = c->fa.armed ? 1 : 0;
     return LLMK_OK;
 }
 
@@ -2109,6 +2253,7 @@
     if (!c || !tokens || n < 1 || pos0 < 1 || pos0 + n - 1 > c->S) return LLMK_E_ARG;
     for (int i = 0; i < n; ++i)
         if (tokens[i] < 0 || tokens[i] > c->V) return LLMK_E_ARG;
+    { const int rc_ = spec_settle(c); if (rc_) return rc_; }
     const int rc = pen_setup(c);
     if (rc) return rc;
     HIPCHK(hipMemcpyAsync(c->d_hist + (pos0 - 1), tokens, (size_t)n * sizeof(int), hipMemcpyHostToDevice, c->stream));
@@ -2117,6 +2262,7 @@
 }
 int llmk_get_history(llmk_ctx* c, int* tokens_out, int n, int pos0) {
     if (!c || !tokens_out || n < 1 || pos0 < 1 || pos0 + n - 1 > c->S) return LLMK_E_ARG;
+    { const int rc_ = spec_settle(c); if (rc_) return rc_; }
     const int rc = pen_setup(c);
     if (rc) return rc;
     HIPCHK(hipMemcpyAsync(tokens_out, c->d_hist + (pos0 - 1), (size_t)n * sizeof(int), hipMemcpyDeviceToHost, c->stream));
@@ -2291,6 +2437,7 @@
     if (!b) return LLMK_E_ARG;
     llmk_ctx* c = b->ctx;
     hipSetDevice(c->cfg.device);
+    { const int rc_ = spec_settle(c); if (rc_) return rc_; }
     hipStreamSynchronize(c->stream);
     --c->n_batches;
     batch_free(b);
@@ -2307,6 +2454,7 @@
     if (!b || slot < 0 || slot >= b->n_slots || n_pos < 0 || n_pos > std::min(b->seq_len, b->ctx->S)) return LLMK_E_ARG;
     llmk_ctx* c = b->ctx;
     HIPCHK(hipSetDevice(c->cfg.device));
+    { const int rc_ = spec_settle(c); if (rc_) return rc_; }
     const size_t row = (size_t)c->KV, slot_rows = (size_t)b->seq_len * row;
     float* caches[2][2] = {{b->d_kc, c->d_kc}, {b->d_vc, c->d_vc}};
     for (auto& p : caches)
@@ -2374,6 +2522,7 @@
     if (b->P < 1) return LLMK_E_STATE;
     llmk_ctx* c = b->ctx;
     HIPCHK(hipSetDevice(c->cfg.device));
+    { const int rc_ = spec_settle(c); if (rc_) return rc_; }
     const size_t slot_rows = (size_t)b->seq_len * c->KV;
     for (float* base : {b->d_kc, b->d_vc})
         for (int l = 0; l < c->L; ++l)
@@ -2601,6 +2750,7 @@
     if (!b || !tokens || slot < 0 || slot >= b->n_slots || n < 1 || pos0 < 1 || pos0 + n - 1 > b->seq_len) return LLMK_E_ARG;
     for (int i = 0; i < n; ++i)
         if (tokens[i] < 0 || tokens[i] > b->ctx->V) return LLMK_E_ARG;
+    { const int rc_ = spec_settle(b->ctx); if (rc_) return rc_; }
     const int rc = rows_pen_setup(b);
     if (rc) return rc;
     hipStream_t st = b->ctx->stream;
@@ -2610,6 +2760,7 @@
 }
 int llmk_rows_get_history(llmk_batch* b, int slot, int* tokens_out, int n, int pos0) {
     if (!b || !tokens_out || slot < 0 || slot >= b->n_slots || n < 1 || pos0 < 1 || pos0 + n - 1 > b->seq_len) return LLMK_E_ARG;
+    { const int rc_ = spec_settle(b->ctx); if (rc_) return rc_; }
     const int rc = rows_pen_setup(b);
     if (rc) return rc;
     hipStream_t st = b->ctx->stream;
@@ -2652,6 +2803,7 @@
 int llmk_reset(llmk_ctx* c) {
     if (!c) return LLMK_E_ARG;
     HIPCHK(hipSetDevice(c->cfg.device));
+    { const int rc = spec_settle(c); if (rc) return rc; }
     const size_t kvn = (size_t)c->L * c->S * c->KVl * sizeof(float);
     HIPCHK(hipMemsetAsync(c->d_kc, 0, kvn, c->stream));
     HIPCHK(hipMemsetAsync(c->d_vc, 0, kvn, c->stream));
@@ -2815,6 +2967,7 @@
 int llmk_peek(llmk_ctx* c, int which, int layer, int pos, float* out, int n) {
     if (!c || !out || n <= 0) return LLMK_E_ARG;
     HIPCHK(hipSetDevice(c->cfg.device));
+    { const int rc = spec_settle(c); if (rc) return rc; }
     const float* src = nullptr;
     int len = 0;
     switch (which) {
@@ -2863,6 +3016,7 @@
     if (!c || !id_in || c->comm) return LLMK_E_ARG;
     if (c->p2p) return LLMK_E_STATE;
     HIPCHK(hipSetDevice(c->cfg.device));
+    { const int rc_ = spec_settle(c); if (rc_) return rc_; }
     ncclUniqueId id;
     memcpy(&id, id_in, sizeof(id));
     if (ncclCommInitRank(&c->comm, c->tp_size, id, c->tp_rank) != ncclSuccess) { c->comm = nullptr; return LLMK_E_COMM; }
@@ -2888,6 +3042,7 @@
 
 int llmk_tp_p2p_handle(llmk_ctx* c, char handle_out[64]) {
     if (!c || !handle_out) return LLMK_E_ARG;
+    { const int rc_ = spec_settle(c); if (rc_) return rc_; }
     int rc = tp_inbox_alloc(c);
     if (rc) return rc;
     static_assert(sizeof(hipIpcMemHandle_t) == 64, "hipIpcMemHandle_t is 64 bytes");
@@ -2899,6 +3054,7 @@
 
 int llmk_tp_p2p_connect(llmk_ctx* c, const char* handles) {
     if (!c || !handles || c->p2p) return LLMK_E_ARG;
+    { const int rc_ = spec_settle(c); if (rc_) return rc_; }
     int rc = tp_inbox_alloc(c);
     if (rc) return rc;
     for (int r = 0; r < c->tp_size; ++r) {
@@ -2916,6 +3072,7 @@
 
 int llmk_tp_p2p_connect_local(llmk_ctx* c, llmk_ctx* const* ranks) {
     if (!c || !ranks || c->p2p) return LLMK_E_ARG;
+    { const int rc_ = spec_settle(c); if (rc_) return rc_; }
     int rc = tp_inbox_alloc(c);
     if (rc) return rc;
     for (int r = 0; r < c->tp_size; ++r) {
@@ -3009,6 +3166,7 @@
 int llmk_tp_p2p_disable(llmk_ctx* c) {
     if (!c) return LLMK_E_ARG;
     HIPCHK(hipSetDevice(c->cfg.device));
+    { const int rc_ = spec_settle(c); if (rc_) return rc_; }
     HIPCHK(hipStreamSynchronize(c->stream));
     c->p2p = false;
     drop_graphs(c);
@@ -3054,18 +3212,21 @@
 int llmk_tp_read_partial(llmk_ctx* c, float* out) {
     if (!c || !out) return LLMK_E_ARG;
     HIPCHK(hipSetDevice(c->cfg.device));
+    { const int rc_ = spec_settle(c); if (rc_) return rc_; }
     HIPCHK(hipMemcpy(out, c->d_part, (size_t)c->E * sizeof(float), hipMemcpyDeviceToHost));
     return LLMK_OK;
 }
 int llmk_tp_write_partial(llmk_ctx* c, const float* in) {
     if (!c || !in) return LLMK_E_ARG;
     HIPCHK(hipSetDevice(c->cfg.device));
+    { const int rc_ = spec_settle(c); if (rc_) return rc_; }
     HIPCHK(hipMemcpy(c->d_part, in, (size_t)c->E * sizeof(float), hipMemcpyHostToDevice));
     return LLMK_OK;
 }
 int llmk_tp_read_logits(llmk_ctx* c, float* out_slice) {
     if (!c || !out_slice) return LLMK_E_ARG;
     HIPCHK(hipSetDevice(c->cfg.device));
+    { const int rc_ = spec_settle(c); if (rc_) return rc_; }
     HIPCHK(hipMemcpy(out_slice, c->d_logits + (size_t)c->tp_rank * c->Vl, (size_t)c->Vl * sizeof(float), hipMemcpyDeviceToHost));
     return LLMK_OK;
 }
@@ -3082,6 +3243,7 @@
     const DevTensor& t = c->t[tid];
     if (!t.data) return LLMK_E_STATE;
     HIPCHK(hipSetDevice(c->cfg.device));
+    { const int rc_ = spec_settle(c); if (rc_) return rc_; }
     const size_t nwords = (size_t)d.rows * (d.layered ? c->L : 1) * t.row_bytes / 4;
     unsigned long long* d_out = nullptr;
     HIPCHK(dev_alloc(&d_out, sizeof(*d_out)));
@@ -3139,6 +3301,7 @@
     if (!c) return LLMK_E_ARG;
     if (c->n_batches > 0) return LLMK_E_STATE;
     hipSetDevice(c->cfg.device);
+    if (c->stream) spec_settle(c);
     if (c->stream) hipStreamSynchronize(c->stream);
     if (c->comm) ncclCommDestroy(c->comm);
     for (int r = 0; r < TP_MAX_RANKS; ++r)
@@ -3165,6 +3328,9 @@
         if (c->q16[i]) hipFree(c->q16[i]);
     if (c->h_tokpos) hipHostFree(c->h_tokpos);
     if (c->h_logits) hipHostFree(c->h_logits);
+    if (c->fa_buf[1]) hipHostFree(c->fa_buf[1]);
+    for (hipEvent_t e : c->fa_ev)
+        if (e) hipEventDestroy(e);
     if (c->h_next) hipHostFree(c->h_next);
     if (c->h_samp) hipHostFree(c->h_samp);
     if (c->h_filt) hipHostFree(c->h_filt);
diff --git a/llm.f90_amd/llmk.py b/llm.f90_amd/llmk.py
--- a/llm.f90_amd/llmk.py
+++ b/llm.f90_amd/llmk.py
@@ -17,7 +17,7 @@
 SYMBOLS = ["llmk_create", "llmk_create_tp", "llmk_tp_unique_id", "llmk_tp_init_comm", "llmk_tp_p2p_handle", "llmk_tp_p2p_connect",
            "llmk_tp_p2p_connect_local", "llmk_tp_p2p_selftest", "llmk_tp_p2p_stress", "llmk_tp_p2p_disable", "llmk_tp_begin", "llmk_tp_segment",
            "llmk_tp_read_partial", "llmk_tp_write_partial", "llmk_tp_read_logits", "llmk_upload", "llmk_upload_rows",
-           "llmk_set_rope_freqs", "llmk_set_tensor_type", "llmk_set_rms_eps", "llmk_forward", "llmk_prefill", "llmk_forward_greedy", "llmk_decode_greedy",
+           "llmk_set_rope_freqs", "llmk_set_tensor_type", "llmk_set_rms_eps", "llmk_forward", "llmk_forward_ahead_stats", "llmk_prefill", "llmk_forward_greedy", "llmk_decode_greedy",
            "llmk_forward_sample", "llmk_decode_sample", "llmk_forward_sample_ex", "llmk_decode_sample_ex", "llmk_sample_logits", "llmk_set_history", "llmk_get_history",
            "llmk_forward_sample_pen", "llmk_decode_sample_pen", "llmk_sample_logits_pen", "llmk_forward_sample_lp", "llmk_decode_sample_lp",
            "llmk_logprob_logits", "llmk_score", "llmk_batch_create", "llmk_batch_destroy", "llmk_batch_fork", "llmk_batch_forward",
@@ -135,6 +135,8 @@
         L.llmk_set_tensor_type.argtypes = [vp, ci, ci]
         L.llmk_set_rms_eps.argtypes = [vp, C.c_float]
         L.llmk_forward.argtypes = [vp, ci, ci, cf]
+        if hasattr(L, "llmk_forward_ahead_stats"):
+            L.llmk_forward_ahead_stats.argtypes = [vp, C.POINTER(ci)]
         L.llmk_prefill.argtypes = [vp, C.POINTER(ci), ci, ci, cf]
         L.llmk_forward_greedy.argtypes = [vp, ci, ci, C.POINTER(ci)]
         L.llmk_decode_greedy.argtypes = [vp, ci, ci, ci, C.POINTER(ci), vp, vp]
@@ -273,6 +275,11 @@
     def forward_raw(self, token: int, pos: int) -> int:
         return lib().llmk_forward(self._h, token, pos, self._logits.ctypes.data_as(C.POINTER(C.c_float)))
 
+    def forward_ahead_stats(self) -> dict:
+        out = (C.c_int * 4)()
+        _ck(lib().llmk_forward_ahead_stats(self._h, out))
+        return {"launches": out[0], "hits": out[1], "misses": out[2], "armed": bool(out[3])}
+
     def prefill(self, tokens, pos0: int = 1) -> np.ndarray:
         t = np.ascontiguousarray(tokens, np.int32)
         _ck(lib().llmk_prefill(self._h, t.ctypes.data_as(C.POINTER(C.c_int)), len(t), pos0,
```

After: 1384 tokens/s, median of 6. 1.5% higher.
